# bminixhofer/zett

Measured on AMD Instinct MI355X. Metric: predicted token-embeddings/sec (full target vocab), higher is better.
Workload: dtype f16

## Files before the change

### zett_amd/csrc/gemm.hip.h

```cpp
#pragma once

#include <hip/hip_runtime.h>
#include <stdint.h>

#include <type_traits>

#ifndef ZETT_GROUP_M
#define ZETT_GROUP_M 4
#endif

namespace zett {

typedef __attribute__((ext_vector_type(16))) float f32x16;
typedef __attribute__((ext_vector_type(4))) float f32x4;
typedef __attribute__((ext_vector_type(8))) __bf16 bf16x8;
typedef __attribute__((ext_vector_type(4))) uint32_t u32x4;

typedef uint16_t bf16_t;
typedef _Float16 f16_t;
typedef __attribute__((ext_vector_type(8))) _Float16 f16x8;

__device__ __forceinline__ float bf16_to_f32(bf16_t v) { return __uint_as_float(((uint32_t)v) << 16); }
__device__ __forceinline__ bf16_t f32_to_bf16(float f) {
    return __builtin_bit_cast(bf16_t, (__bf16)f);
}

template <typename T> __device__ __forceinline__ T to_lo(float v);
template <> __device__ __forceinline__ float to_lo<float>(float v) { return v; }
template <> __device__ __forceinline__ bf16_t to_lo<bf16_t>(float v) { return f32_to_bf16(v); }
template <> __device__ __forceinline__ f16_t to_lo<f16_t>(float v) { return (f16_t)v; }
template <typename T> __device__ __forceinline__ float lo_to_f32(T v);
template <> __device__ __forceinline__ float lo_to_f32<float>(float v) { return v; }
template <> __device__ __forceinline__ float lo_to_f32<bf16_t>(bf16_t v) { return bf16_to_f32(v); }
template <> __device__ __forceinline__ float lo_to_f32<f16_t>(f16_t v) { return (float)v; }
template <typename T> __device__ __forceinline__ uint32_t pack2_lo(float a, float b);
template <> __device__ __forceinline__ uint32_t pack2_lo<bf16_t>(float a, float b) {
    typedef __attribute__((ext_vector_type(2))) float f32x2_t;
    typedef __attribute__((ext_vector_type(2))) __bf16 bf16x2_t;
    const f32x2_t v = {a, b};
    return __builtin_bit_cast(uint32_t, __builtin_convertvector(v, bf16x2_t));
}
template <> __device__ __forceinline__ uint32_t pack2_lo<f16_t>(float a, float b) {
    typedef __attribute__((ext_vector_type(2))) _Float16 h2;
    const h2 v = {(f16_t)a, (f16_t)b};
    return __builtin_bit_cast(uint32_t, v);
}
template <typename T> __device__ __forceinline__ void unpack2_lo(uint32_t u, float& a, float& b);
template <> __device__ __forceinline__ void unpack2_lo<bf16_t>(uint32_t u, float& a, float& b) { a = __uint_as_float(u << 16); b = __uint_as_float(u & 0xffff0000u); }
template <> __device__ __forceinline__ void unpack2_lo<f16_t>(uint32_t u, float& a, float& b) {
    typedef __attribute__((ext_vector_type(2))) _Float16 h2;
    const h2 v = __builtin_bit_cast(h2, u);
    a = (float)v[0]; b = (float)v[1];
}

enum { ACT_NONE = 0, ACT_GELU_TANH = 1, ACT_GELU_ERF = 2 };

__device__ __forceinline__ float gelu_tanh_f(float x) {
#pragma clang fp contract(off)
    const float x3 = (x * x) * x;
    const float u2 = 1.5957691216057308f * __builtin_fmaf(0.044715f, x3, x);
    const float t = 1.0f - 2.0f * __builtin_amdgcn_rcpf(1.0f + __builtin_amdgcn_exp2f(u2 * 1.4426950408889634f));
    return (0.5f * x) * (1.0f + t);
}
__device__ __forceinline__ float erf_as_f(float x) {
#pragma clang fp contract(off)
    const float ax = fabsf(x);
    const float t = __builtin_amdgcn_rcpf(__builtin_fmaf(0.3275911f, ax, 1.0f));
    float p = 1.061405429f;
    p = __builtin_fmaf(p, t, -1.453152027f);
    p = __builtin_fmaf(p, t, 1.421413741f);
    p = __builtin_fmaf(p, t, -0.284496736f);
    p = __builtin_fmaf(p, t, 0.254829592f);
    const float ex = __builtin_amdgcn_exp2f((ax * ax) * -1.4426950408889634f);
    const float y = __builtin_fmaf(-(p * t), ex, 1.0f);
    return copysignf(y, x);
}
__device__ __forceinline__ float gelu_erf_f(float x) {
#pragma clang fp contract(off)
    return (x * 0.5f) * (1.0f + erf_as_f(x * 0.70710678118654752440f));
}

__device__ __forceinline__ float ln_affine(float x, float mean, float rstd, float g, float b) {
#pragma clang fp contract(off)
    return __builtin_fmaf((x - mean) * rstd, g, b);
}

template <int ACT>
__device__ __forceinline__ float epi_value(float acc, float bias, bool has_res, float res, bool has_scale, float sc, float sh) {
#pragma clang fp contract(off)
    float v = acc + bias;
    if (ACT == 1) v = gelu_tanh_f(v);
    else if (ACT == 2) v = gelu_erf_f(v);
    if (has_res) v = v + res;
    if (has_scale) v = __builtin_fmaf(sc, v, sh);
    return v;
}
template <int ACT>
__device__ __forceinline__ float4 epi_value4(float4 a, float4 bias, bool has_res, float4 res, bool has_scale, float4 sc, float4 sh) {
    return make_float4(epi_value<ACT>(a.x, bias.x, has_res, res.x, has_scale, sc.x, sh.x), epi_value<ACT>(a.y, bias.y, has_res, res.y, has_scale, sc.y, sh.y),
                       epi_value<ACT>(a.z, bias.z, has_res, res.z, has_scale, sc.z, sh.z), epi_value<ACT>(a.w, bias.w, has_res, res.w, has_scale, sc.w, sh.w));
}

typedef __attribute__((ext_vector_type(2))) float f32x2;
#define ZETT_PIN_STAGE(arr, n) do { _Pragma("unroll") for (int e_ = 0; e_ < (n); ++e_) asm volatile("" : "+v"((arr)[e_])); } while (0)

template <int ACT, bool HAS_RES, bool HAS_SCALE, int NV>
__device__ __forceinline__ void epi_values(float (&vs)[NV], const float (&bias)[NV], const float (&res)[NV], const float (&sc)[NV], const float (&sh)[NV]) {
#pragma clang fp contract(off)
    static_assert(NV % 2 == 0, "pairs");
    constexpr int NP = NV / 2;
    f32x2 v[NP];
#pragma unroll
    for (int e = 0; e < NP; ++e) v[e] = f32x2{vs[2 * e], vs[2 * e + 1]} + f32x2{bias[2 * e], bias[2 * e + 1]};
    if (ACT == ACT_GELU_TANH) {
        f32x2 u2[NP], t[NP];
        ZETT_PIN_STAGE(v, NP);
#pragma unroll
        for (int e = 0; e < NP; ++e) u2[e] = (v[e] * v[e]) * v[e];
        ZETT_PIN_STAGE(u2, NP);
#pragma unroll
        for (int e = 0; e < NP; ++e) u2[e] = 1.5957691216057308f * __builtin_elementwise_fma(f32x2{0.044715f, 0.044715f}, u2[e], v[e]);
        ZETT_PIN_STAGE(u2, NP);
#pragma unroll
        for (int e = 0; e < NP; ++e) u2[e] = u2[e] * 1.4426950408889634f;
        ZETT_PIN_STAGE(u2, NP);
#pragma unroll
        for (int e = 0; e < NP; ++e) t[e] = f32x2{__builtin_amdgcn_exp2f(u2[e].x), __builtin_amdgcn_exp2f(u2[e].y)};
        ZETT_PIN_STAGE(t, NP);
#pragma unroll
        for (int e = 0; e < NP; ++e) t[e] = 1.0f + t[e];
        ZETT_PIN_STAGE(t, NP);
#pragma unroll
        for (int e = 0; e < NP; ++e) t[e] = f32x2{__builtin_amdgcn_rcpf(t[e].x), __builtin_amdgcn_rcpf(t[e].y)};
        ZETT_PIN_STAGE(t, NP);
#pragma unroll
        for (int e = 0; e < NP; ++e) t[e] = 1.0f - 2.0f * t[e];
        ZETT_PIN_STAGE(t, NP);
#pragma unroll
        for (int e = 0; e < NP; ++e) v[e] = (0.5f * v[e]) * (1.0f + t[e]);
        ZETT_PIN_STAGE(v, NP);
    } else if (ACT == ACT_GELU_ERF) {
        f32x2 z[NP], ax[NP], t[NP], p[NP], ex[NP];
        ZETT_PIN_STAGE(v, NP);
#pragma unroll
        for (int e = 0; e < NP; ++e) z[e] = v[e] * 0.70710678118654752440f;
        ZETT_PIN_STAGE(z, NP);
#pragma unroll
        for (int e = 0; e < NP; ++e) ax[e] = __builtin_elementwise_abs(z[e]);
#pragma unroll
        for (int e = 0; e < NP; ++e) t[e] = __builtin_elementwise_fma(f32x2{0.3275911f, 0.3275911f}, ax[e], f32x2{1.0f, 1.0f});
        ZETT_PIN_STAGE(t, NP);
#pragma unroll
        for (int e = 0; e < NP; ++e) t[e] = f32x2{__builtin_amdgcn_rcpf(t[e].x), __builtin_amdgcn_rcpf(t[e].y)};
        ZETT_PIN_STAGE(t, NP);
#pragma unroll
        for (int e = 0; e < NP; ++e) ex[e] = (ax[e] * ax[e]) * -1.4426950408889634f;
        ZETT_PIN_STAGE(ex, NP);
#pragma unroll
        for (int e = 0; e < NP; ++e) ex[e] = f32x2{__builtin_amdgcn_exp2f(ex[e].x), __builtin_amdgcn_exp2f(ex[e].y)};
        ZETT_PIN_STAGE(ex, NP);
#pragma unroll
        for (int e = 0; e < NP; ++e) p[e] = __builtin_elementwise_fma(f32x2{1.061405429f, 1.061405429f}, t[e], f32x2{-1.453152027f, -1.453152027f});
        ZETT_PIN_STAGE(p, NP);
#pragma unroll
        for (int e = 0; e < NP; ++e) p[e] = __builtin_elementwise_fma(p[e], t[e], f32x2{1.421413741f, 1.421413741f});
        ZETT_PIN_STAGE(p, NP);
#pragma unroll
        for (int e = 0; e < NP; ++e) p[e] = __builtin_elementwise_fma(p[e], t[e], f32x2{-0.284496736f, -0.284496736f});
        ZETT_PIN_STAGE(p, NP);
#pragma unroll
        for (int e = 0; e < NP; ++e) p[e] = __builtin_elementwise_fma(p[e], t[e], f32x2{0.254829592f, 0.254829592f});
        ZETT_PIN_STAGE(p, NP);
#pragma unroll
        for (int e = 0; e < NP; ++e) p[e] = -(p[e] * t[e]);
        ZETT_PIN_STAGE(p, NP);
#pragma unroll
        for (int e = 0; e < NP; ++e) p[e] = __builtin_elementwise_fma(p[e], ex[e], f32x2{1.0f, 1.0f});
        ZETT_PIN_STAGE(p, NP);
#pragma unroll
        for (int e = 0; e < NP; ++e) p[e] = 1.0f + __builtin_elementwise_copysign(p[e], z[e]);
        ZETT_PIN_STAGE(p, NP);
#pragma unroll
        for (int e = 0; e < NP; ++e) v[e] = (v[e] * 0.5f) * p[e];
        ZETT_PIN_STAGE(v, NP);
    }
    if (HAS_RES) {
#pragma unroll
        for (int e = 0; e < NP; ++e) v[e] = v[e] + f32x2{res[2 * e], res[2 * e + 1]};
    }
    if (HAS_SCALE) {
#pragma unroll
        for (int e = 0; e < NP; ++e) v[e] = __builtin_elementwise_fma(f32x2{sc[2 * e], sc[2 * e + 1]}, v[e], f32x2{sh[2 * e], sh[2 * e + 1]});
    }
#pragma unroll
    for (int e = 0; e < NP; ++e) { vs[2 * e] = v[e].x; vs[2 * e + 1] = v[e].y; }
}

template <typename T>
struct GemmEpilogue {
    const float* bias;
    int act;
    const float* residual;
    int ld_res;
    const float* res_stats;
    const float* res_gamma;
    const float* res_beta;
    const int32_t* res_index;
    float2* stats_part;
    int ld_part;
    const float* fold_stats;
    const float* fold_c;
    const float* scale;
    const float* shift;
    float* out_f32;
    int ld_f32;
    T* out_lo;
    int ld_lo;
    int split_col;
    float* out_f32_b;
    int32_t* range_flag;
    int range_final;
    const T* residual_lo;
    int ld_res_lo;
    void* dst;
    const int64_t* dst_rows;
    int64_t ld_dst;
    int dst_dtype;
};

template <typename T> struct LoRange { static constexpr bool checked = false; static constexpr float limit = 0.f; };
template <> struct LoRange<f16_t> { static constexpr bool checked = true; static constexpr float limit = 65504.0f; };
__device__ __forceinline__ bool out_of_range(float v, float limit) { return !(__builtin_fabsf(v) <= limit); }
constexpr float ZETT_F32_MAX = 3.402823466e38f;
constexpr int ZETT_RANGE_BIT_SOURCE = 1, ZETT_RANGE_BIT_ACTIVATION = 2, ZETT_RANGE_BIT_OUTPUT = 4, ZETT_RANGE_BIT_WEIGHT = 8, ZETT_RANGE_BIT_DEST = 16;
template <typename OT> __device__ __forceinline__ bool dest_overflow(float v) {
    if constexpr (std::is_same<OT, f16_t>::value) { const float a = __builtin_fabsf(v); return a >= 65520.0f && a <= 3.402823466e38f; }
    else return false;
// ... 201 lines not shown
```

### zett_amd/csrc/gemm4d.hip.h

```cpp
#pragma once

#include <hip/hip_runtime.h>
#include <stdint.h>

#include <algorithm>
#include <type_traits>

#include "gemm_tile.hip.h"

namespace zett {

#ifndef G4D_ABLATE
#define G4D_ABLATE 5
#endif
constexpr int G4D_ABL = G4D_ABLATE;
#ifdef G4D_MFMA32
constexpr bool G4D_M32 = true;
static_assert(G4D_ABLATE < 5, "the 32x32x16 K loop exists for the ablation levels without an epilogue");
#else
constexpr bool G4D_M32 = false;
#endif
typedef float f32x16 __attribute__((ext_vector_type(16)));

constexpr int g4d_wait_vm(int n) { return ((n >> 4) << 14) | 0x0F70 | (n & 15); }
// ... 14 lines not shown
    asm volatile("v_mfma_f32_32x32x16_f16 %0, %1, %2, %0" : "+a"(c) : "v"(a), "v"(b));
}

template <int K> __device__ __forceinline__ float g4d_xor_lane(float v) {
    return __builtin_bit_cast(float, __builtin_amdgcn_ds_swizzle(__builtin_bit_cast(int, v), (K << 10) | 0x1f));
}


enum { G4D_EPI_GENERIC = 0, G4D_EPI_LO = 1, G4D_EPI_F32 = 2, G4D_EPI_F32_SCALE = 3, G4D_EPI_BOTH = 4, G4D_EPI_F32_LN = 5, G4D_EPI_LO_FOLD = 6,
       G4D_EPI_LO_LN = 7, G4D_EPI_F32_SCALE_FOLD = 8, G4D_EPI_LN16 = 9 };
constexpr int G4D_EPI_STRIDE = 132;
constexpr int G4D_EPI_REGION = 64 * G4D_EPI_STRIDE * 4;
constexpr int G4D_LDS_BYTES = 4 * G4D_EPI_REGION;
static_assert(G4D_LDS_BYTES >= G256_LDS_BYTES && G4D_LDS_BYTES <= 160 * 1024, "LDS budget");

template <bool HALF> struct G4dGeom {
    static constexpr int BM = HALF ? 128 : G256_BM;
    static constexpr int WROWS = BM / 2;
    static constexpr int MI = WROWS / 16;
    static constexpr int AREQ = BM / 32;
    static constexpr int NREQ = AREQ + 8;
    static constexpr int NPASS = WROWS / 64;
    static constexpr int STAGES = HALF ? 3 : 2;
    static constexpr int A_BYTES = BM * GEMM_ROW_BYTES;
    static constexpr int STAGE_BYTES = A_BYTES + G256_OPERAND_BYTES;
    static constexpr int LDS_BYTES = STAGES * STAGE_BYTES;
};

template <typename T, int ACT = ACT_NONE, bool RES = false, int EPI = G4D_EPI_GENERIC, bool HALF = false, typename OT = void>
__global__ __launch_bounds__(256) __attribute__((amdgpu_waves_per_eu(1, 1))) void gemm4d_tn_kernel(GemmArgs<T> g) {
    extern __shared__ __attribute__((aligned(16))) unsigned char smem[];
    constexpr int BK = GEMM_ROW_BYTES / (int)sizeof(T);
    typedef G4dGeom<HALF> GEO;
    static_assert(!HALF || EPI != G4D_EPI_GENERIC, "the half tile carries the streamlined epilogues only");
    constexpr bool DST = !std::is_void<OT>::value;
    static_assert(!DST || EPI == G4D_EPI_F32_SCALE || EPI == G4D_EPI_F32_SCALE_FOLD, "destination stores: the output heads' epilogues only");

    const int tiles_m = (g.M - g.row0 + GEO::BM - 1) / GEO::BM;
    const int tiles_n = (g.N + G256_BN - 1) / G256_BN;
    const int nwg = tiles_m * tiles_n;
    int wg = blockIdx.x;
    {
        const int q = nwg >> 3, r = nwg & 7, xcd = wg & 7;
        wg = (xcd < r ? xcd * (q + 1) : r * (q + 1) + (xcd - r) * q) + (wg >> 3);
    }
    const int GROUP_N = g.group > 0 ? g.group : 4;
    int tm, tn;
    if (g.tile_order == 0) {
        const int group_size = GROUP_N * tiles_m;
        const int first_n = (wg / group_size) * GROUP_N;
        const int gn = (tiles_n - first_n) < GROUP_N ? (tiles_n - first_n) : GROUP_N;
        tn = first_n + (wg % group_size) % gn;
        tm = (wg % group_size) / gn;
    } else {
        const int GROUP_M = g.group > 0 ? g.group : ZETT_GROUP_M;
        const int group_size = GROUP_M * tiles_n;
        const int first_m = (wg / group_size) * GROUP_M;
        const int gm = (tiles_m - first_m) < GROUP_M ? (tiles_m - first_m) : GROUP_M;
        tm = first_m + (wg % group_size) % gm;
        tn = (wg % group_size) / gm;
    }
    const int m0 = g.row0 + tm * GEO::BM, n0 = tn * G256_BN;

    const int tid = threadIdx.x;
    const int lane = tid & 63;
    const int wave = __builtin_amdgcn_readfirstlane(tid >> 6);
    const int wm = wave >> 1, wn = wave & 1;

    const unsigned char* a_base = (const unsigned char*)(g.A + (size_t)m0 * g.lda);
    const unsigned char* w_base = (const unsigned char*)(g.W + (size_t)n0 * g.ldw);
    uint32_t a_voff[8], w_voff[8];
#pragma unroll
    for (int r = 0; r < 8; ++r) {
        const int row = wave * 64 + r * 8 + (lane >> 3);
        const int chunk = ((lane & 7) ^ ((row >> 1) & 7)) << 4;
        int wr = row; wr = n0 + wr < g.N ? wr : g.N - 1 - n0;
        w_voff[r] = (uint32_t)wr * (uint32_t)g.ldw * (uint32_t)sizeof(T) + chunk;
    }
#pragma unroll
    for (int r = 0; r < GEO::AREQ; ++r) {
        const int row = wave * (GEO::AREQ * 8) + r * 8 + (lane >> 3);
        const int chunk = ((lane & 7) ^ ((row >> 1) & 7)) << 4;
        int ar = row; ar = m0 + ar < g.M ? ar : g.M - 1 - m0;
        a_voff[r] = (uint32_t)ar * (uint32_t)g.lda * (uint32_t)sizeof(T) + chunk;
    }
    const __amdgpu_buffer_rsrc_t a_rsrc = __builtin_amdgcn_make_buffer_rsrc((void*)a_base, (short)0, 0x7fffffff, G4R_RSRC_WORD3);
    const __amdgpu_buffer_rsrc_t w_rsrc = __builtin_amdgcn_make_buffer_rsrc((void*)w_base, (short)0, 0x7fffffff, G4R_RSRC_WORD3);
    unsigned char* const my_rows = smem + wave * 64 * GEMM_ROW_BYTES;
    unsigned char* const my_a_rows = smem + wave * (GEO::AREQ * 8) * GEMM_ROW_BYTES;
    auto dma_a = [&](int stage, int kt, int r) {
        __builtin_amdgcn_raw_ptr_buffer_load_lds(a_rsrc, (lds_ptr_t)(my_a_rows + stage * GEO::STAGE_BYTES + r * 8 * GEMM_ROW_BYTES), 16,
                                                 a_voff[r], kt * GEMM_ROW_BYTES, 0, 0);
    };
    auto dma_w = [&](int stage, int kt, int r) {
        __builtin_amdgcn_raw_ptr_buffer_load_lds(w_rsrc, (lds_ptr_t)(my_rows + stage * GEO::STAGE_BYTES + GEO::A_BYTES + r * 8 * GEMM_ROW_BYTES), 16,
                                                 w_voff[r], kt * GEMM_ROW_BYTES, 0, 0);
    };

    constexpr bool M32 = G4D_M32 && !HALF;
    f32x4 acc[8][8];
    f32x16 acc32[4][4];
    if constexpr (M32) {
#pragma unroll
        for (int i = 0; i < 4; ++i)
#pragma unroll
            for (int j = 0; j < 4; ++j)
#pragma unroll
                for (int r = 0; r < 16; ++r) acc32[i][j][r] = 0.f;
    } else {
#pragma unroll
    for (int i = 0; i < GEO::MI; ++i)
#pragma unroll
        for (int j = 0; j < 8; ++j)
#pragma unroll
            for (int r = 0; r < 4; ++r) acc[i][j][r] = 0.f;
    }

    int a_off[2], w_off[2];
    {
        const int l15 = lane & 15, kq = lane >> 4;
        const int swz = (l15 >> 1) & 7;
#pragma unroll
        for (int kb = 0; kb < 2; ++kb) {
            const int c = ((kb * 4 + kq) ^ swz) << 4;
            a_off[kb] = (wm * GEO::WROWS + l15) * GEMM_ROW_BYTES + c;
            w_off[kb] = GEO::A_BYTES + (wn * 128 + l15) * GEMM_ROW_BYTES + c;
        }
    }
    int a_off32[4], w_off32[4];
    if constexpr (M32) {
        const int l31 = lane & 31, kh = lane >> 5;
        const int swz = (l31 >> 1) & 7;
#pragma unroll
        for (int k16 = 0; k16 < 4; ++k16) {
            const int c = ((k16 * 2 + kh) ^ swz) << 4;
            a_off32[k16] = (wm * GEO::WROWS + l31) * GEMM_ROW_BYTES + c;
            w_off32[k16] = GEO::A_BYTES + (wn * 128 + l31) * GEMM_ROW_BYTES + c;
        }
    }
    u32x4 fa[2][8], fw[2][8];
    auto read_a = [&](int stage, int kb, int i) {
        if constexpr (M32) fa[kb][i] = *(const u32x4*)(smem + stage * GEO::STAGE_BYTES + a_off32[kb * 2 + (i >> 2)] + (i & 3) * 32 * GEMM_ROW_BYTES);
        else fa[kb][i] = *(const u32x4*)(smem + stage * GEO::STAGE_BYTES + a_off[kb] + i * 16 * GEMM_ROW_BYTES);
    };
    auto read_w = [&](int stage, int kb, int j) {
        if constexpr (M32) fw[kb][j] = *(const u32x4*)(smem + stage * GEO::STAGE_BYTES + w_off32[kb * 2 + (j >> 2)] + (j & 3) * 32 * GEMM_ROW_BYTES);
        else fw[kb][j] = *(const u32x4*)(smem + stage * GEO::STAGE_BYTES + w_off[kb] + j * 16 * GEMM_ROW_BYTES);
    };

    const int nk = g.K / BK;
    constexpr bool LN16K = EPI == G4D_EPI_LN16;
    uint4 res16[LN16K ? 16 : 1];
    const bool res16_early = LN16K && g.epi.res_index == nullptr;
    auto res16_request = [&](int p, int t) __attribute__((always_inline)) {
        if constexpr (LN16K) {
            int grow = m0 + wm * GEO::WROWS + p * 64 + t * 4 + (lane >> 4);
            grow = grow < g.M ? grow : g.M - 1;
            int gc = n0 + wn * 128 + (lane & 15) * 8;
            gc = gc < g.N ? gc : 0;
            res16[t] = *(const uint4*)(g.epi.residual_lo + (size_t)grow * g.epi.ld_res_lo + gc);
        }
    };
#pragma unroll
    for (int st = 0; st < GEO::STAGES; ++st) {
        if (st < nk) {
#pragma unroll
            for (int r = 0; r < 8; ++r) dma_w(st, st, r);
#pragma unroll
            for (int r = 0; r < GEO::AREQ; ++r) dma_a(st, st, r);
        }
    }
    {
        const int ahead = (nk < GEO::STAGES ? nk : GEO::STAGES) - 1;
        if (ahead >= 2) __builtin_amdgcn_s_waitcnt(g4d_wait_vm(2 * GEO::NREQ));
        else if (ahead == 1) __builtin_amdgcn_s_waitcnt(g4d_wait_vm(GEO::NREQ));
        else __builtin_amdgcn_s_waitcnt(g4d_wait_vm(0));
    }
    __builtin_amdgcn_s_barrier();
    __builtin_amdgcn_sched_barrier(0);
#pragma unroll
    for (int j = 0; j < 8; ++j) read_w(0, 0, j);
#pragma unroll
    for (int i = 0; i < GEO::MI; ++i) read_a(0, 0, i);
    if constexpr (G4D_ABL < 2) {
#pragma unroll
        for (int j = 0; j < 8; ++j) read_w(0, 1, j);
#pragma unroll
        for (int i = 0; i < GEO::MI; ++i) read_a(0, 1, i);
        __builtin_amdgcn_s_waitcnt(G4R_WAIT_LGKM0);
    }

    auto step = [&](int kt, int cur, auto more_c, auto more2_c, auto moreA_c, auto wave_c) {
        constexpr bool more = decltype(more_c)::value, more2 = decltype(more2_c)::value, moreA = decltype(moreA_c)::value;
        constexpr int WV = decltype(wave_c)::value;
        const int nxt = cur + 1 == GEO::STAGES ? 0 : cur + 1;
        constexpr int P_BAR1 = HALF ? 26 : 36, P_BAR2 = HALF ? 52 : 102;
        constexpr int INFLIGHT = HALF ? ((more2 ? 1 : 0) + (moreA ? 1 : 0)) * GEO::NREQ : (moreA ? GEO::NREQ : 0);
#pragma unroll
        for (int kb = 0; kb < 2; ++kb)
#pragma unroll
        for (int i = 0; i < GEO::MI; ++i)
#pragma unroll
        for (int j = 0; j < 8; ++j) {
            const int p = kb * (GEO::MI * 8) + i * 8 + j;
            if (G4D_ABL >= 4 && p == P_BAR1 && (moreA || (!more && EPI != G4D_EPI_GENERIC))) {
                __builtin_amdgcn_s_waitcnt(G4R_WAIT_LGKM0);
                __builtin_amdgcn_s_barrier();
                __builtin_amdgcn_sched_barrier(0);
            }
            if (G4D_ABL >= 4 && p == P_BAR2 && more) {
                __builtin_amdgcn_s_waitcnt(g4d_wait_vm(INFLIGHT));
                __builtin_amdgcn_s_barrier();
                __builtin_amdgcn_sched_barrier(0);
            }
            if constexpr (M32) {
                if ((p & 1) == 0) {
                    const int q = (p >> 1) & 31, h = q >> 4, i32 = (q >> 2) & 3, j32 = q & 3;
                    mfma32_agpr<T>(acc32[i32][j32], fa[kb][h * 4 + i32], fw[kb][h * 4 + j32]);
                }
            } else
            mfma16_agpr<T>(acc[i][j], fa[kb][i], fw[kb][j]);
            constexpr bool RD = G4D_ABL >= 2, DMA = G4D_ABL >= 3;
            if (RD && p < 16 && (p & 1) == 0) read_w(cur, 1, p >> 1);
            if constexpr (!HALF) {
                if (RD && p >= 16 && p <= 30 && (p & 1) == 0) read_a(cur, 1, (p - 16) >> 1);
                if (DMA && moreA && p >= 38 && p < 70 && WV == ((p - 38) & 3)) dma_w(cur, kt + 2, (p - 38) >> 2);
                if (DMA && moreA && p >= 70 && p < 102 && WV == ((p - 70) & 3)) dma_a(cur, kt + 2, (p - 70) >> 2);
                if (RD && more && p >= 103 && p <= 110) read_w(nxt, 0, p - 103);
                if (RD && more && p >= 111 && p <= 125 && (p & 1) == 1) read_a(nxt, 0, (p - 111) >> 1);
                if constexpr (LN16K) { if (!more && p >= 40 && p < 104 && (p & 3) == 0 && res16_early) res16_request(0, (p - 40) >> 2); }
            } else {
                if (p >= 16 && p <= 22 && (p & 1) == 0) read_a(cur, 1, (p - 16) >> 1);
                if (moreA && p >= 27 && p < 43 && (WV & 1) == ((p - 27) & 1)) dma_w(cur, kt + 3, (p - 27) >> 1);
                if (moreA && p >= 43 && p < 51 && (WV & 1) == ((p - 43) & 1)) dma_a(cur, kt + 3, (p - 43) >> 1);
                if (more && p >= 53 && p <= 60) read_w(nxt, 0, p - 53);
                if (more && p >= 60 && p <= 63) read_a(nxt, 0, p - 60);
                if constexpr (LN16K) { if (!more && p >= 24 && p < 56 && (p & 1) == 0 && res16_early) res16_request(0, (p - 24) >> 1); }
            }
            if (!M32 || (p & 1)) __builtin_amdgcn_sched_barrier(0);
        }
    };
    typedef std::integral_constant<bool, true> yes_t;
    typedef std::integral_constant<bool, false> no_t;
    auto k_loop = [&](auto wave_c) {
        int kt = 0, cur = 0;
        auto next = [&]() { ++kt; cur = cur + 1 == GEO::STAGES ? 0 : cur + 1; };
        for (; kt + GEO::STAGES < nk; next()) step(kt, cur, yes_t{}, yes_t{}, yes_t{}, wave_c);
        if constexpr (HALF) {
            if (kt + 2 < nk) { step(kt, cur, yes_t{}, yes_t{}, no_t{}, wave_c); next(); }
        }
        if (kt + 1 < nk) { step(kt, cur, yes_t{}, no_t{}, no_t{}, wave_c); next(); }
        step(kt, cur, no_t{}, no_t{}, no_t{}, wave_c);
    };
    if (wave == 0) k_loop(std::integral_constant<int, 0>{});
    else if (wave == 1) k_loop(std::integral_constant<int, 1>{});
    else if (wave == 2) k_loop(std::integral_constant<int, 2>{});
    else k_loop(std::integral_constant<int, 3>{});

    asm volatile("s_nop 15\n\ts_nop 15");
    if constexpr (G4D_ABL < 5) {
        float keep = 0.f;
        if constexpr (M32) {
#pragma unroll
            for (int i = 0; i < 4; ++i)
#pragma unroll
                for (int j = 0; j < 4; ++j)
#pragma unroll
                    for (int r = 0; r < 16; ++r) keep += acc32[i][j][r];
        } else {
#pragma unroll
        for (int i = 0; i < GEO::MI; ++i)
#pragma unroll
            for (int j = 0; j < 8; ++j) keep += acc[i][j][0] + acc[i][j][1] + acc[i][j][2] + acc[i][j][3];
        }
        if (keep == 123.456f) g.epi.out_lo[threadIdx.x] = (T)0;
        return;
    }
    int tid_e = tid;
    asm volatile("" : "+v"(tid_e));
    const int lane_e = tid_e & 63;
    const int l15 = lane_e & 15, kq = lane_e >> 4;
    if constexpr (EPI == G4D_EPI_GENERIC) {
        __syncthreads();
        float* region = (float*)(smem + wave * 32768);
        typedef EpiDrain<T, ACT, RES, 64, 128, !RES, false> Drain;
        const int gcol = n0 + wn * 128 + (lane_e % Drain::LPR) * 8;
        const bool col_ok = gcol < g.N;
        float4 bias8[2], sc8[2], sh8[2];
        Drain::load_cols(g.epi, gcol, col_ok, bias8, sc8, sh8);
        float4 lng[2], lnb[2];
        Drain::load_ln_cols(g.epi, gcol, col_ok, lng, lnb);
#pragma unroll
        for (int p = 0; p < 2; ++p) {
            float4 oa[Drain::NIT], ob[Drain::NIT];
            const int row0 = m0 + wm * 128 + p * 64;
            Drain::load_res(g, row0, gcol, col_ok, lane_e, oa, ob);
            float2 lnst;
            Drain::load_res_stats(g, row0, lane_e, lnst);
#pragma unroll
            for (int i4 = 0; i4 < 4; ++i4)
#pragma unroll
                for (int j = 0; j < 8; ++j)
#pragma unroll
                    for (int r = 0; r < 4; ++r)
                        region[(i4 * 16 + kq * 4 + r) * 128 + j * 16 + l15] = acc[4 * p + i4][j][r];
            if (RES || p == 0) __builtin_amdgcn_s_waitcnt(GEMM_WAIT_VMCNT0);
            Drain::ln_res(g, lane_e, lng, lnb, lnst, oa, ob);
            Drain::drain(g, region, row0, gcol, col_ok, lane_e, bias8, sc8, sh8, oa, ob);
        }
    } else {
        constexpr bool LO = EPI == G4D_EPI_LO || EPI == G4D_EPI_LO_FOLD, SCALE = EPI == G4D_EPI_F32_SCALE || EPI == G4D_EPI_F32_SCALE_FOLD;
        constexpr bool LN16 = EPI == G4D_EPI_LN16;
        constexpr bool LNP = EPI == G4D_EPI_F32_LN || EPI == G4D_EPI_LO_LN || LN16, FOLD = EPI == G4D_EPI_LO_FOLD || EPI == G4D_EPI_F32_SCALE_FOLD;
        constexpr bool WF32 = EPI != G4D_EPI_LO_LN && !LN16;
        static_assert(!LNP || RES, "a LayerNorm producer is a residual epilogue");
        static_assert((EPI != G4D_EPI_F32_LN && !LN16) || ACT == ACT_NONE, "the encoder's producer has no activation");
        static_assert(!LN16 || sizeof(T) == 2, "16-bit residual stream");
        constexpr int CPL = (LO || LN16) ? 8 : 4;
        constexpr int LPR = 128 / CPL;
        constexpr int RPI = 64 / LPR;
        constexpr int NIT = 64 / RPI;
        static_assert(!(LO && RES), "the 16-bit-only epilogue has no residual");
        float* region = (float*)(smem + wave * G4D_EPI_REGION);
        const GemmEpilogue<T>& e = g.epi;
        constexpr bool W16 = LO || EPI == G4D_EPI_BOTH || LNP;
        constexpr bool CHK16 = W16 && LoRange<T>::checked;
        const bool chk_final = !W16 && e.range_final != 0;
        bool bad = false;
        const int idx = lane_e % LPR, rsub = lane_e / LPR;
        const int gcol = n0 + wn * 128 + idx * CPL;
        const bool col_ok = gcol < g.N;
        const int grow0 = m0 + wm * GEO::WROWS + rsub;
        float bias[CPL], sc[CPL], sh[CPL];
#pragma unroll
        for (int c = 0; c < CPL; ++c) { bias[c] = 0.f; sc[c] = 1.f; sh[c] = 0.f; }
        if (col_ok) {
#pragma unroll
            for (int c4 = 0; c4 < CPL; c4 += 4) {
                if (e.bias) { const float4 b = *(const float4*)(e.bias + gcol + c4); bias[c4] = b.x; bias[c4 + 1] = b.y; bias[c4 + 2] = b.z; bias[c4 + 3] = b.w; }
                if (SCALE) {
                    const float4 a = *(const float4*)(e.scale + gcol + c4), b = *(const float4*)(e.shift + gcol + c4);
                    sc[c4] = a.x; sc[c4 + 1] = a.y; sc[c4 + 2] = a.z; sc[c4 + 3] = a.w;
                    sh[c4] = b.x; sh[c4 + 1] = b.y; sh[c4 + 2] = b.z; sh[c4 + 3] = b.w;
                }
            }
        }
        const bool res_ln = RES && ACT == ACT_NONE && e.res_stats != nullptr;
        float lg[CPL], lb[CPL];
#pragma unroll
        for (int c = 0; c < CPL; ++c) { lg[c] = 1.f; lb[c] = 0.f; }
        float2 pst[2] = {make_float2(0.f, 1.f), make_float2(0.f, 1.f)};
        if constexpr (RES && ACT == ACT_NONE) {
            if (res_ln) {
                if (col_ok) {
#pragma unroll
                    for (int c4 = 0; c4 < CPL; c4 += 4) {
                        const float4 a = *(const float4*)(e.res_gamma + gcol + c4), b = *(const float4*)(e.res_beta + gcol + c4);
                        lg[c4] = a.x; lg[c4 + 1] = a.y; lg[c4 + 2] = a.z; lg[c4 + 3] = a.w; lb[c4] = b.x; lb[c4 + 1] = b.y; lb[c4 + 2] = b.z; lb[c4 + 3] = b.w;
                    }
                }
#pragma unroll
                for (int p = 0; p < GEO::NPASS; ++p) {
                    int srow = m0 + wm * GEO::WROWS + p * 64 + lane_e; srow = srow < g.M ? srow : g.M - 1;
                    if (e.res_index) srow = e.res_index[srow];
                    pst[p] = *(const float2*)(e.res_stats + 2 * (size_t)srow);
                }
            }
        }
        int rix[2] = {0, 0};
        const bool res_ix = RES && e.res_index != nullptr;
        if constexpr (RES) {
            if (res_ix) {
#pragma unroll
                for (int p = 0; p < GEO::NPASS; ++p) {
                    int srow = m0 + wm * GEO::WROWS + p * 64 + lane_e; srow = srow < g.M ? srow : g.M - 1;
                    rix[p] = e.res_index[srow];
                }
            }
        }
        float fc[FOLD ? CPL : 1];
        float2 fst[2] = {make_float2(0.f, 1.f), make_float2(0.f, 1.f)};
        if constexpr (FOLD) {
#pragma unroll
            for (int c = 0; c < CPL; ++c) fc[c] = 0.f;
            if (col_ok) {
#pragma unroll
                for (int c4 = 0; c4 < CPL; c4 += 4) {
                    const float4 a = *(const float4*)(e.fold_c + gcol + c4);
                    fc[c4] = a.x; fc[c4 + 1] = a.y; fc[c4 + 2] = a.z; fc[c4 + 3] = a.w;
                }
            }
#pragma unroll
            for (int p = 0; p < GEO::NPASS; ++p) {
                int srow = m0 + wm * GEO::WROWS + p * 64 + lane_e; srow = srow < g.M ? srow : g.M - 1;
                fst[p] = *(const float2*)(e.fold_stats + 2 * (size_t)srow);
            }
        }
        int64_t drow[2] = {0, 0};
        if constexpr (DST) {
#pragma unroll
            for (int p = 0; p < GEO::NPASS; ++p) {
                int srow = m0 + wm * GEO::WROWS + p * 64 + lane_e; srow = srow < g.M ? srow : g.M - 1;
                drow[p] = e.dst_rows ? e.dst_rows[srow] : (int64_t)srow;
            }
        }
        bool bad_dst = false;
        constexpr int RB = LNP ? 1 : 2;
        float4 res[LN16 ? 1 : RB][(RES && !LN16) ? NIT : 1];
        auto load_res16 = [&](int p, int ta, int tb) {
            if constexpr (LN16) {
#pragma unroll
                for (int t = ta; t < tb; ++t) {
                    if (res_ix) {
                        const int grow = grow0 + p * 64 + t * RPI;
                        const size_t rrow = (size_t)__shfl(rix[p], t * RPI + rsub, 64);
                        res16[t] = (grow < g.M && col_ok) ? *(const uint4*)(e.residual_lo + rrow * e.ld_res_lo + gcol) : make_uint4(0u, 0u, 0u, 0u);
                    } else {
                        res16_request(p, t);
                    }
                }
            }
        };
        auto load_res = [&](int p) {
            if constexpr (LN16) {
                load_res16(p, 0, NIT);
            } else if constexpr (RES) {
#pragma unroll
                for (int t = 0; t < NIT; ++t) {
                    const int grow = grow0 + p * 64 + t * RPI;
                    size_t rrow = (size_t)grow;
                    if (res_ix) {
                        const int i0 = __builtin_amdgcn_readlane(rix[p], t * RPI), i1 = __builtin_amdgcn_readlane(rix[p], t * RPI + 1);
                        rrow = (size_t)(rsub ? i1 : i0);
                    }
                    res[p % RB][t] = (grow < g.M && col_ok) ? *(const float4*)(e.residual + rrow * e.ld_res + gcol) : make_float4(0.f, 0.f, 0.f, 0.f);
                }
            }
        };
        auto stage = [&](int p) {
#pragma unroll
            for (int i4 = 0; i4 < 4; ++i4)
#pragma unroll
                for (int j = 0; j < 8; ++j)
#pragma unroll
                    for (int r = 0; r < 4; ++r)
                        region[(i4 * 16 + kq * 4 + r) * G4D_EPI_STRIDE + j * 16 + l15] = acc[4 * p + i4][j][r];
            if constexpr (FOLD)
                *(float2*)(region + lane_e * G4D_EPI_STRIDE + 128) = fst[p];
            if constexpr (LN16)
                *(float2*)(region + lane_e * G4D_EPI_STRIDE + 128) = pst[p];
        };
        auto drain = [&](int p, auto full_c) {
            constexpr bool FULL = decltype(full_c)::value;
            constexpr int GROUP = (LO || RES) ? 4 : 8;
            constexpr int NV = GROUP * CPL;
            float acc_s = 0.f, acc_q = 0.f;
#pragma unroll
            for (int t0 = 0; t0 < NIT; t0 += GROUP) {
                float v[NV], bb[NV], rr[NV], ss[NV], hh[NV];
#pragma unroll
                for (int u = 0; u < GROUP; ++u) {
                    const float* src = region + ((t0 + u) * RPI + rsub) * G4D_EPI_STRIDE + idx * CPL;
#pragma unroll
                    for (int c4 = 0; c4 < CPL; c4 += 4) {
                        const float4 x = *(const float4*)(src + c4);
                        v[u * CPL + c4] = x.x; v[u * CPL + c4 + 1] = x.y; v[u * CPL + c4 + 2] = x.z; v[u * CPL + c4 + 3] = x.w;
                    }
#pragma unroll
                    for (int c = 0; c < CPL; ++c) { bb[u * CPL + c] = bias[c]; ss[u * CPL + c] = sc[c]; hh[u * CPL + c] = sh[c]; rr[u * CPL + c] = 0.f; }
                    if constexpr (LN16) {
                        const uint4 x = res16[t0 + u];
                        unpack2_lo<T>(x.x, rr[u * 8], rr[u * 8 + 1]); unpack2_lo<T>(x.y, rr[u * 8 + 2], rr[u * 8 + 3]);
                        unpack2_lo<T>(x.z, rr[u * 8 + 4], rr[u * 8 + 5]); unpack2_lo<T>(x.w, rr[u * 8 + 6], rr[u * 8 + 7]);
                        if (res_ln) {
                            const float2 st = *(const float2*)(region + ((t0 + u) * RPI + rsub) * G4D_EPI_STRIDE + 128);
#pragma unroll
                            for (int c = 0; c < 8; ++c) rr[u * 8 + c] = ln_affine(rr[u * 8 + c], st.x, st.y, lg[c], lb[c]);
                        }
                    } else if constexpr (RES) {
                        const float4 x = res[p % RB][t0 + u];
                        rr[u * CPL] = x.x; rr[u * CPL + 1] = x.y; rr[u * CPL + 2] = x.z; rr[u * CPL + 3] = x.w;
                        if (ACT == ACT_NONE && res_ln) {
                            const int r0 = (t0 + u) * RPI;
                            const float mean0 = __builtin_bit_cast(float, __builtin_amdgcn_readlane(__builtin_bit_cast(int, pst[p].x), r0));
                            const float mean1 = __builtin_bit_cast(float, __builtin_amdgcn_readlane(__builtin_bit_cast(int, pst[p].x), r0 + 1));
                            const float rstd0 = __builtin_bit_cast(float, __builtin_amdgcn_readlane(__builtin_bit_cast(int, pst[p].y), r0));
                            const float rstd1 = __builtin_bit_cast(float, __builtin_amdgcn_readlane(__builtin_bit_cast(int, pst[p].y), r0 + 1));
                            const float mean = rsub ? mean1 : mean0, rstd = rsub ? rstd1 : rstd0;
#pragma unroll
                            for (int c = 0; c < 4; ++c) rr[u * CPL + c] = ln_affine(rr[u * CPL + c], mean, rstd, lg[c], lb[c]);
                        }
                    }
                }
                if constexpr (FOLD) {
#pragma unroll
                    for (int u = 0; u < GROUP; ++u) {
                        const float2 st = *(const float2*)(region + ((t0 + u) * RPI + rsub) * G4D_EPI_STRIDE + 128);
                        const float t = -st.x * st.y;
                        const f32x2 t2 = {t, t}, r2 = {st.y, st.y};
#pragma unroll
                        for (int c = 0; c < CPL; c += 2) {
                            const f32x2 x = __builtin_elementwise_fma(t2, f32x2{fc[c], fc[c + 1]}, f32x2{bias[c], bias[c + 1]});
                            const f32x2 y = __builtin_elementwise_fma(f32x2{v[u * CPL + c], v[u * CPL + c + 1]}, r2, x);
                            v[u * CPL + c] = y.x; v[u * CPL + c + 1] = y.y;
                            bb[u * CPL + c] = 0.f; bb[u * CPL + c + 1] = 0.f;
                        }
                    }
                }
                epi_values<ACT, RES, SCALE, NV>(v, bb, rr, ss, hh);
                if constexpr (CHK16) {
#pragma unroll
                    for (int x = 0; x < NV; ++x) bad |= out_of_range(v[x], LoRange<T>::limit);
                } else if (chk_final) {
#pragma unroll
                    for (int x = 0; x < NV; ++x) bad |= out_of_range(v[x], ZETT_F32_MAX);
                }
                if constexpr (LN16) {
                    static_assert(!LN16 || (GROUP == 4 && CPL == 8 && RPI == 4), "reduce-scatter layout");
                    float S[4], Q[4];
#pragma unroll
                    for (int u = 0; u < 4; ++u) {
                        const float* x = v + 8 * u;
                        S[u] = ((x[0] + x[1]) + (x[2] + x[3])) + ((x[4] + x[5]) + (x[6] + x[7]));
                        Q[u] = __builtin_fmaf(x[0], x[0], __builtin_fmaf(x[1], x[1], __builtin_fmaf(x[2], x[2], __builtin_fmaf(x[3], x[3],
                               __builtin_fmaf(x[4], x[4], __builtin_fmaf(x[5], x[5], __builtin_fmaf(x[6], x[6], x[7] * x[7])))))));
                    }
                    const bool b3 = (idx & 8) != 0, b2 = (idx & 4) != 0;
                    float ks0 = b3 ? S[2] : S[0], ks1 = b3 ? S[3] : S[1], kq0 = b3 ? Q[2] : Q[0], kq1 = b3 ? Q[3] : Q[1];
                    ks0 += g4d_xor_lane<8>(b3 ? S[0] : S[2]); ks1 += g4d_xor_lane<8>(b3 ? S[1] : S[3]);
                    kq0 += g4d_xor_lane<8>(b3 ? Q[0] : Q[2]); kq1 += g4d_xor_lane<8>(b3 ? Q[1] : Q[3]);
                    float ks = b2 ? ks1 : ks0, kq = b2 ? kq1 : kq0;
                    ks += g4d_xor_lane<4>(b2 ? ks0 : ks1); kq += g4d_xor_lane<4>(b2 ? kq0 : kq1);
                    ks += g4d_xor_lane<2>(ks); kq += g4d_xor_lane<2>(kq);
                    ks += g4d_xor_lane<1>(ks); kq += g4d_xor_lane<1>(kq);
                    const bool mine = (idx & 3) == (t0 >> 2);
                    acc_s = mine ? ks : acc_s; acc_q = mine ? kq : acc_q;
                } else if constexpr (LNP) {
                    static_assert(GROUP == 4 && CPL == 4 && RPI == 2, "reduce-scatter layout");
                    float S[4], Q[4];
#pragma unroll
                    for (int u = 0; u < 4; ++u) {
                        const float a = v[4 * u], b = v[4 * u + 1], c = v[4 * u + 2], d = v[4 * u + 3];
                        S[u] = (a + b) + (c + d);
                        Q[u] = __builtin_fmaf(a, a, __builtin_fmaf(b, b, __builtin_fmaf(c, c, d * d)));
                    }
                    const bool b4 = (idx & 16) != 0, b3 = (idx & 8) != 0;
                    float ks0 = b4 ? S[2] : S[0], ks1 = b4 ? S[3] : S[1], kq0 = b4 ? Q[2] : Q[0], kq1 = b4 ? Q[3] : Q[1];
                    ks0 += g4d_xor_lane<16>(b4 ? S[0] : S[2]); ks1 += g4d_xor_lane<16>(b4 ? S[1] : S[3]);
                    kq0 += g4d_xor_lane<16>(b4 ? Q[0] : Q[2]); kq1 += g4d_xor_lane<16>(b4 ? Q[1] : Q[3]);
                    float ks = b3 ? ks1 : ks0, kq = b3 ? kq1 : kq0;
                    ks += g4d_xor_lane<8>(b3 ? ks0 : ks1); kq += g4d_xor_lane<8>(b3 ? kq0 : kq1);
                    ks += g4d_xor_lane<4>(ks); kq += g4d_xor_lane<4>(kq);
                    ks += g4d_xor_lane<2>(ks); kq += g4d_xor_lane<2>(kq);
                    ks += g4d_xor_lane<1>(ks); kq += g4d_xor_lane<1>(kq);
                    const bool mine = (idx & 7) == (t0 >> 2);
                    acc_s = mine ? ks : acc_s; acc_q = mine ? kq : acc_q;
                }
#pragma unroll
                for (int u = 0; u < GROUP; ++u) {
                    const int grow = grow0 + p * 64 + (t0 + u) * RPI;
                    if (!FULL && (grow >= g.M || !col_ok)) continue;
                    if constexpr (LO || LN16) {
                        const float4 a = make_float4(v[u * 8], v[u * 8 + 1], v[u * 8 + 2], v[u * 8 + 3]);
                        const float4 b = make_float4(v[u * 8 + 4], v[u * 8 + 5], v[u * 8 + 6], v[u * 8 + 7]);
                        store_out8<T>(e.out_lo + (size_t)grow * e.ld_lo + gcol, a, b);
                    } else {
                        const f32x4 x = {v[u * 4], v[u * 4 + 1], v[u * 4 + 2], v[u * 4 + 3]};
                        if constexpr (DST) {
                            const int r0 = (t0 + u) * RPI;
                            static_assert(!DST || RPI == 2, "two rows per instruction");
                            const uint64_t d64 = (uint64_t)drow[p];
                            const uint32_t lo0 = __builtin_amdgcn_readlane((uint32_t)d64, r0), hi0 = __builtin_amdgcn_readlane((uint32_t)(d64 >> 32), r0);
                            const uint32_t lo1 = __builtin_amdgcn_readlane((uint32_t)d64, r0 + 1), hi1 = __builtin_amdgcn_readlane((uint32_t)(d64 >> 32), r0 + 1);
                            const int64_t d = (int64_t)(((uint64_t)(rsub ? hi1 : hi0) << 32) | (rsub ? lo1 : lo0));
                            if (d >= 0) {
                                store_out4<OT>((OT*)e.dst + d * e.ld_dst + gcol, make_float4(x[0], x[1], x[2], x[3]));
#pragma unroll
                                for (int c = 0; c < 4; ++c) bad_dst |= dest_overflow<OT>(x[c]);
                            }
                        } else if constexpr (WF32) {
                            float* d = e.out_f32 + (size_t)grow * e.ld_f32 + gcol;
                            if (RES) asm volatile("global_store_dwordx4 %0, %1, off nt\n\ts_nop 1" :: "v"(d), "v"(x) : "memory");
                            else *(f32x4*)d = x;
                        }
                        if constexpr (EPI == G4D_EPI_BOTH || LNP)
                            store_out4<T>(e.out_lo + (size_t)grow * e.ld_lo + gcol, make_float4(x[0], x[1], x[2], x[3]));
                    }
                }
                if constexpr (LN16 && GEO::NPASS == 2) { if (p == 0 && t0 == GROUP) load_res16(1, 0, NIT / 2); }
            }
            if constexpr (LN16 && GEO::NPASS == 2) { if (p == 0) load_res16(1, NIT / 2, NIT); }
            if constexpr (LNP) {
                const int rp = LN16 ? (((4 * (idx & 3) + 2 * ((idx >> 3) & 1) + ((idx >> 2) & 1)) << 2) + rsub)
                                    : (((4 * (idx & 7) + 2 * ((idx >> 4) & 1) + ((idx >> 3) & 1)) << 1) + rsub);
                const int grow = m0 + wm * GEO::WROWS + p * 64 + rp;
                if (grow < g.M && n0 + wn * 128 < g.N)
                    e.stats_part[(size_t)((n0 + wn * 128) >> 7) * e.ld_part + grow] = make_float2(acc_s, acc_q);
            }
        };
        auto drain_pass = [&](int p) {
            const bool full = m0 + wm * GEO::WROWS + p * 64 + 64 <= g.M && n0 + wn * 128 + 128 <= g.N;
            if (full) drain(p, std::integral_constant<bool, true>{});
            else drain(p, std::integral_constant<bool, false>{});
        };
        if constexpr (LN16) { if (!res16_early) load_res(0); }
        else load_res(0);
        stage(0);
        __builtin_amdgcn_sched_barrier(0);
        if constexpr (!LNP && GEO::NPASS == 2) load_res(1);
        __builtin_amdgcn_sched_barrier(0);
        drain_pass(0);
        if constexpr (GEO::NPASS == 2) {
            if constexpr (LNP && !LN16) { __builtin_amdgcn_sched_barrier(0); load_res(1); __builtin_amdgcn_sched_barrier(0); }
            stage(1);
            drain_pass(1);
        }
        range_report(e.range_flag, bad, W16 ? ZETT_RANGE_BIT_ACTIVATION : ZETT_RANGE_BIT_OUTPUT);
        if constexpr (DST) range_report(e.range_flag, bad_dst, ZETT_RANGE_BIT_DEST);
    }
}

template <typename T>
inline int gemm4d_epi_mode(const GemmArgs<T>& g) {
    const GemmEpilogue<T>& e = g.epi;
    if (e.stats_part && e.residual_lo) {
        if (sizeof(T) == 2 && e.out_lo && !e.out_f32 && !e.residual && e.act == ACT_NONE && !e.scale && !e.shift && !e.out_f32_b && e.split_col >= g.N &&
            g.N % 128 == 0 && e.ld_lo % 8 == 0 && e.ld_res_lo % 8 == 0) return G4D_EPI_LN16;
        return -1;
    }
    if (e.stats_part) {
        const bool common = e.out_lo && e.residual && !e.scale && !e.shift && !e.out_f32_b && e.split_col >= g.N && g.N % 128 == 0 &&
                            e.ld_lo % 4 == 0 && e.ld_res % 4 == 0;
        if (common && e.out_f32 && e.act == ACT_NONE && e.ld_f32 % 4 == 0) return G4D_EPI_F32_LN;
        if (common && !e.out_f32 && e.act == ACT_GELU_TANH && !e.res_stats && !e.res_index) return G4D_EPI_LO_LN;
        return -1;
    }
    if (e.fold_stats) {
        if (e.fold_c && e.out_lo && !e.out_f32 && !e.residual && !e.scale && !e.shift && !e.out_f32_b && e.split_col >= g.N &&
            g.N % 8 == 0 && e.ld_lo % 8 == 0) return G4D_EPI_LO_FOLD;
        if (e.fold_c && e.out_f32 && !e.out_lo && !e.residual && e.scale && e.shift && e.act == ACT_NONE && !e.out_f32_b && e.split_col >= g.N &&
            g.N % 4 == 0 && e.ld_f32 % 4 == 0) return G4D_EPI_F32_SCALE_FOLD;
        return -1;
    }
    if (e.out_f32_b || e.split_col < g.N) return G4D_EPI_GENERIC;
    if (e.res_stats && (e.act != ACT_NONE || !e.residual)) return G4D_EPI_GENERIC;
    if (e.out_lo && !e.out_f32 && !e.residual && !e.scale && !e.shift && g.N % 8 == 0 && e.ld_lo % 8 == 0) return G4D_EPI_LO;
    if (e.out_f32 && e.out_lo && !e.residual && !e.scale && !e.shift && e.act == ACT_NONE && g.N % 4 == 0 && e.ld_f32 % 4 == 0 && e.ld_lo % 4 == 0)
        return G4D_EPI_BOTH;
    if (e.out_f32 && !e.out_lo && g.N % 4 == 0 && e.ld_f32 % 4 == 0 && (!e.residual || e.ld_res % 4 == 0)) {
        if (e.scale && e.shift && !e.residual && e.act == ACT_NONE) return G4D_EPI_F32_SCALE;
        if (!e.scale && !e.shift && (e.act == ACT_NONE || (e.act == ACT_GELU_TANH && e.residual))) return G4D_EPI_F32;
    }
    return G4D_EPI_GENERIC;
}

template <typename T, int ACT, bool RES, int EPI, bool HALF = false>
inline hipError_t launch_gemm4d_inst(const GemmArgs<T>& g, hipStream_t stream) {
    constexpr int lds = EPI == G4D_EPI_GENERIC ? G256_LDS_BYTES : (G4dGeom<HALF>::LDS_BYTES > G4D_LDS_BYTES ? G4dGeom<HALF>::LDS_BYTES : G4D_LDS_BYTES);
    static_assert(lds <= 160 * 1024, "LDS budget");
    static DeviceFlags attr;
    bool* done = attr.current();
    if (!done || !*done) {
        hipError_t e = hipFuncSetAttribute((const void*)gemm4d_tn_kernel<T, ACT, RES, EPI, HALF>, hipFuncAttributeMaxDynamicSharedMemorySize, lds);
        if (e != hipSuccess) return e;
        if (done) *done = true;
    }
    constexpr int BM = HALF ? 128 : G256_BM;
    const int tiles_m = (g.M - g.row0 + BM - 1) / BM;
    const int tiles_n = (g.N + G256_BN - 1) / G256_BN;
    if (tiles_m <= 0 || tiles_n <= 0) return hipSuccess;
    hipLaunchKernelGGL((gemm4d_tn_kernel<T, ACT, RES, EPI, HALF>), dim3(tiles_m * tiles_n), dim3(256), lds, stream, g);
    return hipGetLastError();
}

template <typename T, int ACT, bool HALF>
inline hipError_t launch_gemm4d_act(const GemmArgs<T>& g, hipStream_t stream, int mode) {
    const bool res = g.epi.residual != nullptr;
    switch (mode) {
        case G4D_EPI_LO: return launch_gemm4d_inst<T, ACT, false, G4D_EPI_LO, HALF>(g, stream);
        case G4D_EPI_LO_FOLD: return launch_gemm4d_inst<T, ACT, false, G4D_EPI_LO_FOLD, HALF>(g, stream);
        case G4D_EPI_F32:
            if constexpr (ACT == ACT_NONE) return res ? launch_gemm4d_inst<T, ACT, true, G4D_EPI_F32, HALF>(g, stream) : launch_gemm4d_inst<T, ACT, false, G4D_EPI_F32, HALF>(g, stream);
            else if constexpr (ACT == ACT_GELU_TANH) { if (res) return launch_gemm4d_inst<T, ACT, true, G4D_EPI_F32, HALF>(g, stream); }
            [[fallthrough]];
        default:
            if constexpr (HALF) return hipErrorInvalidValue;
            else return res ? launch_gemm4d_inst<T, ACT, true, G4D_EPI_GENERIC>(g, stream) : launch_gemm4d_inst<T, ACT, false, G4D_EPI_GENERIC>(g, stream);
    }
}

template <typename T, bool HALF>
inline hipError_t launch_gemm4d_mode(const GemmArgs<T>& g, hipStream_t stream, int mode) {
    if (mode == G4D_EPI_F32_LN) return launch_gemm4d_inst<T, ACT_NONE, true, G4D_EPI_F32_LN, HALF>(g, stream);
    if (mode == G4D_EPI_LN16) return launch_gemm4d_inst<T, ACT_NONE, true, G4D_EPI_LN16, HALF>(g, stream);
    if (mode == G4D_EPI_LO_LN) return launch_gemm4d_inst<T, ACT_GELU_TANH, true, G4D_EPI_LO_LN, HALF>(g, stream);
    if (mode == G4D_EPI_F32_SCALE_FOLD) return launch_gemm4d_inst<T, ACT_NONE, false, G4D_EPI_F32_SCALE_FOLD, HALF>(g, stream);
    if (mode == G4D_EPI_F32_SCALE) return launch_gemm4d_inst<T, ACT_NONE, false, G4D_EPI_F32_SCALE, HALF>(g, stream);
    if (mode == G4D_EPI_BOTH) return launch_gemm4d_inst<T, ACT_NONE, false, G4D_EPI_BOTH, HALF>(g, stream);
    switch (g.epi.act) {
        case ACT_GELU_TANH: return launch_gemm4d_act<T, ACT_GELU_TANH, HALF>(g, stream, mode);
        case ACT_GELU_ERF: return launch_gemm4d_act<T, ACT_GELU_ERF, HALF>(g, stream, mode);
        default: return launch_gemm4d_act<T, ACT_NONE, HALF>(g, stream, mode);
    }
}

template <typename T>
inline bool gemm4d_half_ok(const GemmArgs<T>& g, int mode) {
    if (mode <= G4D_EPI_GENERIC) return false;
    if (mode == G4D_EPI_F32) return g.epi.act == ACT_NONE || (g.epi.act == ACT_GELU_TANH && g.epi.residual);
    return true;
}

inline int gemm4d_row_split(int M, int N, int cus = 256, double half_cost = 0.62) {
    const long tn = (N + G256_BN - 1) / G256_BN, tm = (M + G256_BM - 1) / G256_BM;
    const long T = tm * tn;
    if (T % cus == 0) return M;
    const long rounds = (T + cus - 1) / cus;
    const long tm_full = std::min<long>(tm, ((rounds - 1) * cus) / tn);
    const long row0 = tm_full * G256_BM;
    if (row0 >= M) return M;
    const long th = ((M - row0 + 127) / 128) * tn;
    const double cost = (double)((tm_full * tn + cus - 1) / cus) + half_cost * (double)((th + cus - 1) / cus);
    return cost < (double)rounds - 0.05 ? (int)row0 : M;
}

template <typename T, int EPI, typename OT, bool HALF>
inline hipError_t launch_gemm4d_dst_inst(const GemmArgs<T>& g, hipStream_t stream) {
    constexpr int lds = G4dGeom<HALF>::LDS_BYTES > G4D_LDS_BYTES ? G4dGeom<HALF>::LDS_BYTES : G4D_LDS_BYTES;
    static DeviceFlags attr;
    bool* done = attr.current();
    if (!done || !*done) {
        hipError_t e = hipFuncSetAttribute((const void*)gemm4d_tn_kernel<T, ACT_NONE, false, EPI, HALF, OT>, hipFuncAttributeMaxDynamicSharedMemorySize, lds);
        if (e != hipSuccess) return e;
        if (done) *done = true;
    }
    constexpr int BM = HALF ? 128 : G256_BM;
    const int tiles_m = (g.M - g.row0 + BM - 1) / BM;
    const int tiles_n = (g.N + G256_BN - 1) / G256_BN;
    if (tiles_m <= 0 || tiles_n <= 0) return hipSuccess;
    hipLaunchKernelGGL((gemm4d_tn_kernel<T, ACT_NONE, false, EPI, HALF, OT>), dim3(tiles_m * tiles_n), dim3(256), lds, stream, g);
    return hipGetLastError();
}

template <typename T, bool HALF>
inline hipError_t launch_gemm4d_dst_mode(const GemmArgs<T>& g, hipStream_t stream, int mode) {
    const int dt = g.epi.dst_dtype;
    if (mode == G4D_EPI_F32_SCALE_FOLD) {
        if (dt == 1) return launch_gemm4d_dst_inst<T, G4D_EPI_F32_SCALE_FOLD, f16_t, HALF>(g, stream);
        if (dt == 2) return launch_gemm4d_dst_inst<T, G4D_EPI_F32_SCALE_FOLD, bf16_t, HALF>(g, stream);
        return launch_gemm4d_dst_inst<T, G4D_EPI_F32_SCALE_FOLD, float, HALF>(g, stream);
    }
    if (dt == 1) return launch_gemm4d_dst_inst<T, G4D_EPI_F32_SCALE, f16_t, HALF>(g, stream);
    if (dt == 2) return launch_gemm4d_dst_inst<T, G4D_EPI_F32_SCALE, bf16_t, HALF>(g, stream);
    return launch_gemm4d_dst_inst<T, G4D_EPI_F32_SCALE, float, HALF>(g, stream);
}

template <typename T>
inline int gemm4d_dst_mode(const GemmArgs<T>& g) {
    const GemmEpilogue<T>& e = g.epi;
    if (!e.dst || e.dst_dtype < 0 || e.dst_dtype > 2 || e.ld_dst % 4 != 0) return -1;
    const size_t align = e.dst_dtype == 0 ? 16 : 8;
    if ((uintptr_t)e.dst % align) return -1;
    GemmArgs<T> f = g;
    f.epi.out_f32 = (float*)e.dst;
    f.epi.ld_f32 = 4;
    const int mode = gemm4d_epi_mode(f);
    return (mode == G4D_EPI_F32_SCALE || mode == G4D_EPI_F32_SCALE_FOLD) ? mode : -1;
}

hipError_t launch_gemm_4d_half(const GemmArgs<f16_t>& g, hipStream_t stream, int mode);
hipError_t launch_gemm_4d_half(const GemmArgs<bf16_t>& g, hipStream_t stream, int mode);

hipError_t launch_gemm_4d_half_dst(const GemmArgs<f16_t>& g, hipStream_t stream, int mode);
hipError_t launch_gemm_4d_half_dst(const GemmArgs<bf16_t>& g, hipStream_t stream, int mode);

template <typename T>
inline hipError_t launch_gemm4d(const GemmArgs<T>& g, hipStream_t stream, bool force_generic = false) {
    const bool dst = g.epi.dst != nullptr;
    const int mode = dst ? gemm4d_dst_mode(g) : (force_generic && !g.epi.stats_part && !g.epi.fold_stats) ? G4D_EPI_GENERIC : gemm4d_epi_mode(g);
    if (mode < 0) return hipErrorInvalidValue;
    int split = g.row0 == -1 ? gemm4d_row_split(g.M, g.N) : (g.row0 == -2 ? 0 : (g.row0 > 0 ? std::min(g.row0, g.M) : g.M));
    if (split < g.M && (!gemm4d_half_ok(g, mode) || split % G256_BM != 0)) split = g.M;
    GemmArgs<T> full = g;
    full.row0 = 0;
    if (split < g.M) {
        full.M = split;
        if (split > 0)
            if (hipError_t e = dst ? launch_gemm4d_dst_mode<T, false>(full, stream, mode) : launch_gemm4d_mode<T, false>(full, stream, mode); e != hipSuccess) return e;
        GemmArgs<T> rest = g;
        rest.row0 = split;
        return dst ? launch_gemm_4d_half_dst(rest, stream, mode) : launch_gemm_4d_half(rest, stream, mode);
    }
    return dst ? launch_gemm4d_dst_mode<T, false>(full, stream, mode) : launch_gemm4d_mode<T, false>(full, stream, mode);
}

}
```

### zett_amd/csrc/rowops.hip.h

```cpp
#pragma once

#include <hip/hip_runtime.h>
#include <stdint.h>

#include <type_traits>

#include "gemm.hip.h"

namespace zett {


struct PlanArrays {
    int32_t* row_count;
    int32_t* row_offset;
    uint8_t* row_uniform;
    int32_t* id_flag;
    int32_t* id_slot;
    int32_t* id_list;
    int32_t* tok_slot;
    int32_t* tok_pos;
    int32_t* tok_row;
    int32_t* tok_pkey;
    int32_t* pair_flag;
    int32_t* pair_slot;
// ... 600 lines not shown

struct AttentionWaves { int64_t total, full; int full_groups, lanes_per_row; };
__host__ __device__ inline AttentionWaves attention_waves(int rows, int H, bool pack) {
    const int rem = H & 511, gfull = H >> 9;
    AttentionWaves a;
    if (pack && (rem == 256 || rem == 128 || rem == 64)) {
        a.full_groups = gfull; a.lanes_per_row = rem >> 3;
        a.full = (int64_t)rows * gfull;
        const int per = 64 / a.lanes_per_row;
        a.total = a.full + (rows + per - 1) / per;
    } else {
        a.full_groups = (H + 511) >> 9; a.lanes_per_row = 64;
        a.full = (int64_t)rows * a.full_groups;
        a.total = a.full;
    }
    return a;
}

template <typename T>
__global__ __launch_bounds__(256) void attention_rows_kernel(const T* __restrict__ qbase, size_t ldq,
                                                             const T* __restrict__ kbase, const T* __restrict__ vbase,
                                                             size_t ldkv, int H, int head_dim,
                                                             const int32_t* __restrict__ row_offset,
                                                             const uint8_t* __restrict__ row_uniform,
                                                             const uint8_t* __restrict__ tok_key, int64_t row0,
                                                             int rows, int tok0, float scaling, int flags ,
                                                             const int32_t* __restrict__ tok_pair, T* __restrict__ ctx) {
    const int cls_only = flags & 1;
    const int lane = threadIdx.x & 63;
    const int64_t w = (int64_t)blockIdx.x * 4 + (threadIdx.x >> 6);
    const AttentionWaves aw = attention_waves(rows, H, (flags & 4) != 0);
    if (w >= aw.total) return;
    int rl, grp, li = lane, base = 0, lpr = 64;
    bool valid = true;
    if (w < aw.full) { rl = (int)(w / aw.full_groups); grp = (int)(w % aw.full_groups); }
    else {
        lpr = aw.lanes_per_row;
        const int sub = lane / lpr;
        li = lane - sub * lpr;
        base = sub * lpr;
        rl = (int)(w - aw.full) * (64 / lpr) + sub;
        grp = aw.full_groups;
        valid = rl < rows;
        if (!valid) rl = rows - 1;
    }
    const int col = grp * 512 + li * 8;
    const bool active = valid && col < H;
    const int lph = head_dim >> 3;
    const int64_t n = row0 + rl;
    const int t0 = row_offset[n] - tok0, t1 = row_offset[n + 1] - tok0;
    const bool uniform = row_uniform[n];
    const int nq = cls_only ? 1 : (t1 - t0);
    const int ccol = active ? col : 0;
    auto brow = [&](int t) -> size_t { return (size_t)chunk_row(t, rl, t == t0, rows); };
    int pslot = 0;
    if (tok_pair) { const int t = t0 + li; pslot = t < t1 ? tok_pair[tok0 + t] : 0; }
    auto qrow = [&](int t) -> size_t {
        if (!tok_pair) return brow(t);
        return t - t0 < lpr ? (size_t)__shfl(pslot, base + (t - t0), 64) : (size_t)tok_pair[tok0 + t];
    };
    const int nk = t1 - t0;
    if constexpr (sizeof(T) == 2) {
        if (nk <= ATT_FAST_KEYS && (flags & 2)) {
            const bool mine = li < nk && (uniform || tok_key[tok0 + t0 + li] != 0);
            const unsigned on = (unsigned)(__ballot(mine) >> base) & (lpr >= 32 ? 0xffffffffu : ((1u << lpr) - 1u));
            uint4 kk[ATT_FAST_KEYS], vv[ATT_FAST_KEYS], qq[ATT_FAST_KEYS];
#pragma unroll
            for (int j = 0; j < ATT_FAST_KEYS; ++j) {
                if (j < nk) {
                    const size_t kr = qrow(t0 + j);
                    kk[j] = *(const uint4*)(kbase + kr * ldkv + ccol);
                    vv[j] = *(const uint4*)(vbase + kr * ldkv + ccol);
                    if (!cls_only) qq[j] = *(const uint4*)(qbase + kr * ldq + ccol);
                }
            }
            if (cls_only) qq[0] = *(const uint4*)(qbase + (size_t)rl * ldq + ccol);
            const float sc2 = scaling * 1.4426950408889634f;
#pragma unroll
            for (int qi = 0; qi < ATT_FAST_KEYS; ++qi) {
                if (qi < nq) {
                    float sj[ATT_FAST_KEYS];
                    float mx = -INFINITY;
#pragma unroll
                    for (int j = 0; j < ATT_FAST_KEYS; ++j) {
                        sj[j] = -INFINITY;
                        if (j < nk && ((on >> j) & 1u)) {
                            const float d = head_sum(dot8_lo<T>(qq[qi], kk[j]), lph);
                            sj[j] = uniform ? 0.f : d * sc2;
                            mx = fmaxf(mx, sj[j]);
                        }
                    }
                    float l = 0.f, acc[8];
#pragma unroll
                    for (int c = 0; c < 8; ++c) acc[c] = 0.f;
#pragma unroll
                    for (int j = 0; j < ATT_FAST_KEYS; ++j) {
                        if (j < nk && ((on >> j) & 1u)) {
                            const float pj = __builtin_amdgcn_exp2f(sj[j] - mx);
                            l += pj;
                            float v[8];
                            unpack2_lo<T>(vv[j].x, v[0], v[1]); unpack2_lo<T>(vv[j].y, v[2], v[3]);
                            unpack2_lo<T>(vv[j].z, v[4], v[5]); unpack2_lo<T>(vv[j].w, v[6], v[7]);
#pragma unroll
                            for (int c = 0; c < 8; ++c) acc[c] = fmaf(pj, v[c], acc[c]);
                        }
                    }
                    const float inv = 1.0f / l;
#pragma unroll
                    for (int c = 0; c < 8; ++c) acc[c] *= inv;
                    if (active) {
                        const size_t orow = cls_only ? (size_t)rl : brow(t0 + qi);
                        store8<T>(ctx + orow * H + col, acc);
                    }
                }
            }
            return;
        }
    }
    for (int qi = 0; qi < nq; ++qi) {
        float q[8];
        load8<T>(qbase + (cls_only ? (size_t)rl : qrow(t0 + qi)) * ldq + ccol, q);
        float mx = -INFINITY, l = 0.f, acc[8];
#pragma unroll
        for (int c = 0; c < 8; ++c) acc[c] = 0.f;
        for (int kj = t0; kj < t1; ++kj) {
            if (!uniform && !tok_key[tok0 + kj]) continue;
            float k[8], v[8];
            const size_t kr = qrow(kj);
            load8<T>(kbase + kr * ldkv + ccol, k);
            load8<T>(vbase + kr * ldkv + ccol, v);
            float s = 0.f;
#pragma unroll
            for (int c = 0; c < 8; ++c) s = fmaf(q[c], k[c], s);
            for (int off = 1; off < lph; off <<= 1) s += __shfl_xor(s, off, 64);
            s = uniform ? 0.f : s * scaling;
            const float nm = fmaxf(mx, s);
            const float corr = expf(mx - nm);
            const float p = expf(s - nm);
            l = fmaf(l, corr, p);
#pragma unroll
            for (int c = 0; c < 8; ++c) acc[c] = fmaf(acc[c], corr, p * v[c]);
            mx = nm;
        }
        const float inv = 1.0f / l;
#pragma unroll
        for (int c = 0; c < 8; ++c) acc[c] *= inv;
        if (active) {
            const size_t orow = cls_only ? (size_t)rl : brow(t0 + qi);
            store8<T>(ctx + orow * H + col, acc);
        }
    }
}

__global__ __launch_bounds__(64) void ln_stats_kernel(const float2* __restrict__ part, int parts, int ld_part, int rows, int H, float eps,
                                                      float* __restrict__ stats) {
    const int r = blockIdx.x * blockDim.x + threadIdx.x;
    if (r >= rows) return;
    float s = 0.f, q = 0.f;
    const float2* col = part + r;
    int p = 0;
    for (; p + 8 <= parts; p += 8) {
        float2 v[8];
#pragma unroll
        for (int j = 0; j < 8; ++j) v[j] = col[(size_t)(p + j) * ld_part];
#pragma unroll
        for (int j = 0; j < 8; ++j) { s += v[j].x; q += v[j].y; }
    }
    {
        float2 v[8];
#pragma unroll
        for (int j = 0; j < 8; ++j) v[j] = p + j < parts ? col[(size_t)(p + j) * ld_part] : make_float2(0.f, 0.f);
#pragma unroll
        for (int j = 0; j < 8; ++j)
            if (p + j < parts) { s += v[j].x; q += v[j].y; }
    }
    const float mean = s / (float)H;
    const float var = fmaxf(q / (float)H - mean * mean, 0.f);
    *(float2*)(stats + 2 * (size_t)r) = make_float2(mean, 1.0f / sqrtf(var + eps));
}

template <typename T>
__global__ __launch_bounds__(256) void fold_weight_kernel(const float* __restrict__ w, int K, const float* __restrict__ gamma,
                                                          const float* __restrict__ beta, const float* __restrict__ bias,
                                                          T* __restrict__ w_fold, float* __restrict__ c_out, float* __restrict__ b_out,
                                                          int32_t* __restrict__ range_flag) {
    __shared__ float red[4];
    const int n = blockIdx.x;
    const float* row = w + (size_t)n * K;
    float cs = 0.f, bs = 0.f;
    for (int k = threadIdx.x; k < K; k += 256) {
        const float x = row[k];
        if (LoRange<T>::checked) range_report(range_flag, out_of_range(x * gamma[k], LoRange<T>::limit), ZETT_RANGE_BIT_WEIGHT);
        const T lo = to_lo<T>(x * gamma[k]);
        w_fold[(size_t)n * K + k] = lo;
        cs += lo_to_f32<T>(lo);
        bs = fmaf(x, beta[k], bs);
    }
    const float ct = block_sum_256(cs, red);
    const float bt = block_sum_256(bs, red);
    if (threadIdx.x == 0) { c_out[n] = ct; b_out[n] = bias[n] + bt; }
}

template <typename T>
__global__ void convert_f32_to_lo_kernel(const float* __restrict__ in, T* __restrict__ out, size_t n, int32_t* __restrict__ range_flag) {
    size_t i = ((size_t)blockIdx.x * blockDim.x + threadIdx.x) * 4;
    const size_t stride = (size_t)gridDim.x * blockDim.x * 4;
    bool bad = false;
    for (; i + 3 < n; i += stride) {
        const float4 v = *(const float4*)(in + i);
        if (LoRange<T>::checked)
            bad |= out_of_range(v.x, LoRange<T>::limit) | out_of_range(v.y, LoRange<T>::limit) | out_of_range(v.z, LoRange<T>::limit) |
                   out_of_range(v.w, LoRange<T>::limit);
        store_lo4<T>(out + i, v);
    }
    if (blockIdx.x == 0 && threadIdx.x == 0) {
        for (size_t j = n & ~(size_t)3; j < n; ++j) { out[j] = to_lo<T>(in[j]); if (LoRange<T>::checked) bad |= out_of_range(in[j], LoRange<T>::limit); }
    }
    range_report(range_flag, bad, ZETT_RANGE_BIT_WEIGHT);
}
template <int SRC_DTYPE>
__global__ void convert_to_f32_kernel(const void* __restrict__ in, float* __restrict__ out, size_t n) {
    size_t i = (size_t)blockIdx.x * blockDim.x + threadIdx.x;
    const size_t stride = (size_t)gridDim.x * blockDim.x;
    for (; i < n; i += stride) {
        if constexpr (SRC_DTYPE == 1) out[i] = (float)((const _Float16*)in)[i];
        else out[i] = __uint_as_float(((uint32_t)((const uint16_t*)in)[i]) << 16);
    }
}

template <typename OT> __device__ __forceinline__ void store4_dst(OT* d, float4 v) {
    if constexpr (std::is_same<OT, float>::value) *(float4*)d = v;
    else *(uint2*)d = make_uint2(pack2_lo<OT>(v.x, v.y), pack2_lo<OT>(v.z, v.w));
}

template <typename OT, bool VEC>
__global__ __launch_bounds__(256) void dest_store_rows_kernel(const float* __restrict__ src, int64_t ld_src, OT* __restrict__ dst, int64_t ld_dst,
                                                              const int64_t* __restrict__ rows, int64_t n_rows, int cols, int32_t* range_flag) {
    bool bad = false;
    for (int64_t i = blockIdx.x; i < n_rows; i += gridDim.x) {
        const int64_t d = rows ? rows[i] : i;
        if (d < 0) continue;
        const float* s = src + i * ld_src;
        OT* o = dst + d * ld_dst;
        if constexpr (VEC) {
            for (int c = (int)threadIdx.x * 4; c < cols; c += 256 * 4) {
                const float4 v = *(const float4*)(s + c);
                store4_dst<OT>(o + c, v);
                bad |= dest_overflow<OT>(v.x) | dest_overflow<OT>(v.y) | dest_overflow<OT>(v.z) | dest_overflow<OT>(v.w);
            }
        } else {
            for (int c = (int)threadIdx.x; c < cols; c += 256) {
                const float v = s[c];
                o[c] = to_lo<OT>(v);
                bad |= dest_overflow<OT>(v);
            }
        }
    }
    range_report(range_flag, bad, ZETT_RANGE_BIT_DEST);
}

__global__ void dest_rows_check_kernel(const int64_t* __restrict__ rows, int64_t n, int64_t n_dest, int32_t* err) {
    const int64_t i = (int64_t)blockIdx.x * blockDim.x + threadIdx.x;
    if (i < n && rows[i] >= n_dest) atomicMax(err, (int)(i < 0x7ffffffe ? i + 1 : 0x7fffffff));
}

}
```

### zett_amd/csrc/zett_hip.hip

```cpp
#include <hip/hip_runtime.h>

#include <algorithm>
#include <array>
#include <cstdlib>
#include <cmath>
#include <cstdarg>
#include <cstdio>
#include <cstring>
#include <map>
#include <string>
#include <type_traits>
#include <vector>

#include "../../include/zett_hip.h"
#include "common.hip.h"
#include "gemm.hip.h"
#include "gemm_launch.hip.h"
#include "rowops.hip.h"
#include "retok.hip.h"
#include "lexical.hip.h"
#include "partition.hip.h"

using namespace zett;

namespace {

struct Tensor {
    float* f32 = nullptr;
    void* lo = nullptr;
    std::vector<int64_t> shape;
    size_t numel = 0;
};

inline size_t round_up(size_t v, size_t m) { return (v + m - 1) / m * m; }

}

struct zett_hypernet {
    zett_config cfg{};
    int device = 0;
    int precision = ZETT_PREC_BF16;
    bool finalized = false;
    std::map<std::string, Tensor> w;
    std::vector<void*> qkv_w;
    std::vector<float*> qkv_b;
    struct Folded { void* w = nullptr; float* c = nullptr; float* b = nullptr; };
    std::vector<Folded> fold_qkv, fold_up;
    Folded fold_head_in, fold_head_out;
    float* head_one = nullptr;
    float* head_zero = nullptr;
    int ln_fold = 1;
    float* head_scale = nullptr;
    float* head_shift = nullptr;
    std::vector<void*> owned;
    int64_t max_chunk_tokens = 0;
    int time_gemm = 0;
    int cls_only_last = 1;
    int pair_dedupe = 1;
    int residual_lo = 1;
    int concurrent_lanes = 0;
    hipStream_t lane_stream = nullptr;
    hipEvent_t lane_ev[4] = {nullptr, nullptr, nullptr, nullptr};
    int attention_fast = 1;
    int attention_pack = 1;
    int gemm_tail_split = 1;
    int gemm_tile_order = 0;
    int ln_rows8 = 1;
    int table_lo = 1;
    int gemm_group = 0;
    int gemm4d_min_k = 512;
    int gemm_variant = 0;
    struct PlanSlot {
        DevBuf i32, u8;
        int32_t* host = nullptr;
        size_t host_ints = 0;
        hipEvent_t done = nullptr;
        hipEvent_t released = nullptr;
        const int32_t* sfm = nullptr;
        int64_t n_rows = 0;
        int seq = 0;
        bool pair_plan = false;
        const int32_t* ext_id_slot = nullptr;
        bool pending = false;
    } plan[2];
    PlanSlot table_plan;
    struct ExtTable { const void* table = nullptr; const float* stats = nullptr; const int32_t* id_slot = nullptr; } ext;
    int plan_cur = 0;
    hipStream_t plan_stream = nullptr;
    hipEvent_t plan_fork = nullptr;
    DevBuf table, x0, yf, yt, big, pre, ctx, cf, ct, lnstats, lnparts;
    hipEvent_t out_ready[2] = {nullptr, nullptr};
    bool out_recorded = false;
    int range_accumulate = 0;
    int32_t* range_word = nullptr;
    int32_t* range_host = nullptr;
    DevBuf dest_word, dest_stage[2], dest_sink;
    int32_t* dest_host = nullptr;
    hipEvent_t dest_checked = nullptr;
    std::vector<hipEvent_t> ev;
    size_t ev_used = 0;
    std::vector<double> ev_flops;
    std::vector<std::array<int, 4>> ev_shape;
    std::vector<zett_gemm_record> gemm_log;
    zett_stats stats{};
};

namespace {

size_t elt_size(int precision) { return precision == ZETT_PREC_F32 ? 4 : 2; }

bool is_gemm_weight(const std::string& n) {
    static const char* suffixes[] = {"input_projection.0.weight", "dense1.weight", "dense2.weight",
                                     "query.weight", "key.weight", "value.weight", "dense.weight",
                                     "output_projection.1.weight", "output_projection_out.1.weight"};
    for (const char* s : suffixes) {
        const size_t ls = strlen(s);
        if (n.size() >= ls && n.compare(n.size() - ls, ls, s) == 0) return true;
    }
    return false;
}

void expected_shapes(const zett_config& c, std::map<std::string, std::vector<int64_t>>& s) {
    const int64_t H = c.hidden, I = c.intermediate;
    auto proj = [&](const std::string& p) {
        s[p + "dense1.weight"] = {I, H}; s[p + "dense1.bias"] = {I};
        s[p + "dense2.weight"] = {H, I}; s[p + "dense2.bias"] = {H};
        s[p + "ln.weight"] = {H}; s[p + "ln.bias"] = {H};
    };
    if (c.embed_lang) s["lang_embeddings.weight"] = {c.n_langs, H};
    s["model.embeddings.token_type_embeddings.weight"] = {1, H};
    s["model.embeddings.LayerNorm.weight"] = {H};
    s["model.embeddings.LayerNorm.bias"] = {H};
    s["model.embeddings.position_embeddings.weight"] = {c.max_positions, H};
    for (int l = 0; l < c.layers; ++l) {
        const std::string p = "model.encoder.layer." + std::to_string(l) + ".";
        for (const char* q : {"query", "key", "value"}) {
            s[p + "attention.self." + q + ".weight"] = {H, H};
            s[p + "attention.self." + q + ".bias"] = {H};
        }
        s[p + "attention.output.dense.weight"] = {H, H}; s[p + "attention.output.dense.bias"] = {H};
        s[p + "attention.output.LayerNorm.weight"] = {H}; s[p + "attention.output.LayerNorm.bias"] = {H};
        s[p + "intermediate.dense.weight"] = {I, H}; s[p + "intermediate.dense.bias"] = {I};
        s[p + "output.dense.weight"] = {H, I}; s[p + "output.dense.bias"] = {H};
        s[p + "output.LayerNorm.weight"] = {H}; s[p + "output.LayerNorm.bias"] = {H};
    }
    s["fallback_embeddings.weight"] = {c.n_extra, c.n_in_embd};
    s["input_projection.0.weight"] = {H, c.n_in_embd}; s["input_projection.0.bias"] = {H};
    proj("input_projection.1.");
    proj("output_projection.0.");
    const int64_t w0 = c.single_head ? c.n_in_embd : c.n_embd;
    s["output_projection.1.weight"] = {w0, H}; s["output_projection.1.bias"] = {w0};
    if (c.separate_out && !c.single_head) {
        proj("output_projection_out.0.");
        s["output_projection_out.1.weight"] = {c.n_embd, H}; s["output_projection_out.1.bias"] = {c.n_embd};
    }
    if (c.rescale) {
        s["in_scaler.w"] = {1, c.n_in_embd}; s["in_scaler.b"] = {1, c.n_in_embd};
        s["scaler.w"] = {1, c.n_embd}; s["scaler.b"] = {1, c.n_embd};
        if (c.separate_out) { s["out_scaler.w"] = {1, c.n_embd}; s["out_scaler.b"] = {1, c.n_embd}; }
    }
    if (c.predict_bias) { s["bias_projection.weight"] = {1, H}; s["bias_projection.bias"] = {1}; }
}

int validate_config(const zett_config& c, int precision) {
    if (c.n_embd <= 0 || c.hidden <= 0 || c.intermediate <= 0 || c.heads <= 0 || c.layers <= 0)
        return fail(ZETT_E_INVALID, "non-positive dimension in zett_config");
    if (c.n_in_embd != (c.separate_out ? 2 * c.n_embd : c.n_embd))
        return fail(ZETT_E_INVALID, "n_in_embd must be 2*n_embd iff separate_out");
    if (c.hidden % c.heads) return fail(ZETT_E_INVALID, "hidden %d not divisible by heads %d", c.hidden, c.heads);
    const int d = c.hidden / c.heads;
    if (d < 8 || d > 512 || (d & (d - 1))) return fail(ZETT_E_INVALID, "head_dim %d unsupported (need a power of two in [8,512])", d);
    const int kq = precision == ZETT_PREC_F32 ? 32 : 64;
    for (int k : {c.n_in_embd, c.hidden, c.intermediate})
        if (k % kq) return fail(ZETT_E_INVALID, "contraction width %d is not a multiple of %d", k, kq);
    if (c.n_embd % 4) return fail(ZETT_E_INVALID, "n_embd must be a multiple of 4");
    if (c.n_extra < 1) return fail(ZETT_E_INVALID, "n_extra must be >= 1 (reference allocates max(hn_n_extra_tokens,1))");
    if (c.pad_token_id < 0) return fail(ZETT_E_INVALID, "pad_token_id is required");
    if (c.embed_lang && c.n_langs <= 0) return fail(ZETT_E_INVALID, "hn_embed_lang_id needs n_langs");
    return 0;
}

struct WorkspaceSizes {
    int64_t chunk_tokens;
    size_t table, x0, f32_rows, lo_rows, big, stats;
    size_t total() const { return table + x0 + 3 * f32_rows + 3 * lo_rows + big + stats; }
};

static int64_t pair_keys(const zett_config& c, int seq) {
    return ((int64_t)c.original_vocab_size + c.n_extra + 1) * (int64_t)(seq + (c.embed_lang ? 1 : 0));
}

static size_t plan_i32_bytes(const zett_config& c, int64_t N, int seq) {
    const int64_t V = (int64_t)c.original_vocab_size + c.n_extra;
    const int64_t max_tok = N * (int64_t)(seq + (c.embed_lang ? 1 : 0));
    const int64_t K = pair_keys(c, seq);
    const size_t scan_scratch = 2 * ((size_t)std::max<int64_t>(std::max<int64_t>(N, V), K) / SCAN_CHUNK + 2) + 1;
    return ((size_t)N + (N + 1) + 3 + V + (V + 1) + V + 7 * (size_t)max_tok + 2 * (size_t)K + 2 + scan_scratch) * 4;
}

static int64_t chunk_token_cap(const zett_config& c, size_t es) {
    const size_t wide = (size_t)std::max(c.intermediate, 3 * c.hidden);
    const size_t per_token = (size_t)c.n_in_embd * es + 3 * (size_t)c.hidden * 4 + 3 * (size_t)c.hidden * es + wide * es + 24;
    return std::max<int64_t>(131072, (int64_t)(((size_t)12 << 30) / per_token));
}

static WorkspaceSizes workspace_sizes(const zett_config& c, size_t es, int seq, int64_t Ttot, int64_t D, int64_t cap) {
    const int lam = c.embed_lang ? 1 : 0;
    WorkspaceSizes w{};
    if (cap <= 0) cap = chunk_token_cap(c, es);
    w.chunk_tokens = std::max<int64_t>(std::min<int64_t>(cap, std::max<int64_t>(Ttot, D)), seq + lam);
    const size_t MC = (size_t)w.chunk_tokens, MCS = MC + 768;
    const size_t wide = (size_t)std::max(c.intermediate, 3 * c.hidden);
    w.table = (size_t)D * c.hidden * 4;
    w.x0 = MCS * c.n_in_embd * es;
    w.f32_rows = MCS * c.hidden * 4;
    w.lo_rows = MCS * c.hidden * es;
    w.big = MCS * wide * es;
    w.stats = 2 * MCS * 2 * sizeof(float);
    return w;
}
// ... 83 lines not shown

template <typename T>
int do_forward(zett_hypernet* h, const int32_t* sfm, int64_t N, int seq, const void* src, int src_dtype, const zett_dest* dest,
               int64_t v_src, int lang_index, float* out_in, float* out_out, float* out_bias, hipStream_t st);
template <typename T>
int do_table_rows(zett_hypernet* h, const int32_t* id_list, int first, int count, const void* src, int src_dtype, void* table_out, float* stats_out, hipStream_t st);

}

extern "C" {

const char* zett_last_error(void) { return g_err.c_str(); }
int zett_abi_version(void) { return ZETT_ABI_VERSION; }

int zett_create(const zett_config* cfg, int device, int precision, zett_hypernet** out) {
    if (!cfg || !out) return fail(ZETT_E_INVALID, "null argument");
    if (precision != ZETT_PREC_BF16 && precision != ZETT_PREC_F32 && precision != ZETT_PREC_F16) return fail(ZETT_E_INVALID, "unknown precision %d", precision);
    if (int rc = validate_config(*cfg, precision)) return rc;
    int ndev = 0;
    HIP_TRY(hipGetDeviceCount(&ndev));
    if (device < 0 || device >= ndev) return fail(ZETT_E_INVALID, "device %d out of range (%d visible)", device, ndev);
    ZETT_ON_DEVICE(device);
    auto* h = new zett_hypernet();
    h->cfg = *cfg;
    h->device = device;
    h->precision = precision;
    if (hipMalloc((void**)&h->range_word, 64) != hipSuccess || hipHostMalloc((void**)&h->range_host, 64, hipHostMallocDefault) != hipSuccess ||
        hipMemset(h->range_word, 0, 64) != hipSuccess) {
        if (h->range_word) (void)hipFree(h->range_word);
        if (h->range_host) (void)hipHostFree(h->range_host);
        delete h;
        return fail(ZETT_E_HIP, "allocation of the range word failed");
    }
    *out = h;
    return 0;
}

int zett_destroy(zett_hypernet* h) {
    if (!h) return 0;
    ::zett::DeviceScope _scope(h->device);
    for (auto& kv : h->w) {
        if (kv.second.f32) (void)hipFree(kv.second.f32);
        if (kv.second.lo && kv.second.lo != (void*)kv.second.f32) (void)hipFree(kv.second.lo);
    }
    for (void* p : h->owned) (void)hipFree(p);
    for (DevBuf* b : {&h->table, &h->x0, &h->yf, &h->yt, &h->big, &h->pre, &h->ctx, &h->cf, &h->ct, &h->lnstats, &h->lnparts, &h->dest_word, &h->dest_stage[0], &h->dest_stage[1], &h->dest_sink})
        b->release();
    for (zett_hypernet::PlanSlot* psp : {&h->plan[0], &h->plan[1], &h->table_plan}) {
        zett_hypernet::PlanSlot& ps = *psp;
        ps.i32.release(); ps.u8.release();
        if (ps.host) (void)hipHostFree(ps.host);
        if (ps.done) (void)hipEventDestroy(ps.done);
        if (ps.released) (void)hipEventDestroy(ps.released);
    }
    if (h->plan_stream) (void)hipStreamDestroy(h->plan_stream);
    if (h->plan_fork) (void)hipEventDestroy(h->plan_fork);
    if (h->range_word) (void)hipFree(h->range_word);
    if (h->range_host) (void)hipHostFree(h->range_host);
    if (h->dest_host) (void)hipHostFree(h->dest_host);
    if (h->dest_checked) (void)hipEventDestroy(h->dest_checked);
    for (hipEvent_t e : h->out_ready) if (e) (void)hipEventDestroy(e);
    for (hipEvent_t e : h->lane_ev) if (e) (void)hipEventDestroy(e);
    if (h->lane_stream) (void)hipStreamDestroy(h->lane_stream);
    for (hipEvent_t e : h->ev) (void)hipEventDestroy(e);
    delete h;
    return 0;
}

int zett_load_weight(zett_hypernet* h, const char* name, const void* data, int dtype, const int64_t* shape, int ndim) {
    if (!h || !name || !data || !shape || ndim < 1) return fail(ZETT_E_INVALID, "null argument");
    if (h->finalized) return fail(ZETT_E_STATE, "weights are frozen after zett_finalize");
    std::map<std::string, std::vector<int64_t>> exp;
    expected_shapes(h->cfg, exp);
    const std::string n(name);
    auto it = exp.find(n);
    if (it == exp.end()) return 0;
    std::vector<int64_t> got(shape, shape + ndim);
    if (got != it->second) {
        std::string a, b;
        for (auto v : got) a += std::to_string(v) + ",";
        for (auto v : it->second) b += std::to_string(v) + ",";
        return fail(ZETT_E_INVALID, "%s: shape [%s] does not match the config's [%s]", name, a.c_str(), b.c_str());
    }
    ZETT_ON_DEVICE(h->device);
    size_t numel = 1;
    for (auto v : got) numel *= (size_t)v;
    Tensor& t = h->w[n];
    if (t.f32) { (void)hipFree(t.f32); t.f32 = nullptr; }
    t.shape = got;
    t.numel = numel;
    HIP_TRY(hipMalloc((void**)&t.f32, numel * 4));
    if (dtype == ZETT_F32) {
        HIP_TRY(hipMemcpy(t.f32, data, numel * 4, hipMemcpyDefault));
    } else if (dtype == ZETT_F16 || dtype == ZETT_BF16) {
        void* stage = nullptr;
        HIP_TRY(hipMalloc(&stage, numel * 2));
        hipError_t e = hipMemcpy(stage, data, numel * 2, hipMemcpyDefault);
        if (e == hipSuccess) {
            const int blocks = (int)std::min<size_t>((numel + 255) / 256, 65535);
            if (dtype == ZETT_F16) hipLaunchKernelGGL(convert_to_f32_kernel<1>, dim3(blocks), dim3(256), 0, 0, stage, t.f32, numel);
            else hipLaunchKernelGGL(convert_to_f32_kernel<2>, dim3(blocks), dim3(256), 0, 0, stage, t.f32, numel);
            e = hipDeviceSynchronize();
        }
        (void)hipFree(stage);
        if (e != hipSuccess) return fail(ZETT_E_HIP, "upload of %s failed: %s", name, hipGetErrorString(e));
    } else {
        return fail(ZETT_E_INVALID, "unknown dtype %d", dtype);
    }
    return 0;
}

int zett_finalize(zett_hypernet* h) {
    if (!h) return fail(ZETT_E_INVALID, "null handle");
    if (h->finalized) return 0;
    ZETT_ON_DEVICE(h->device);
    std::map<std::string, std::vector<int64_t>> exp;
    expected_shapes(h->cfg, exp);
    for (auto& kv : exp)
        if (!h->w.count(kv.first)) return fail(ZETT_E_STATE, "missing weight: %s", kv.first.c_str());
    const zett_config& c = h->cfg;
    const size_t es = elt_size(h->precision);
    for (auto& kv : h->w) {
        Tensor& t = kv.second;
        if (!is_gemm_weight(kv.first)) continue;
        if (h->precision == ZETT_PREC_F32) { t.lo = t.f32; continue; }
        HIP_TRY(hipMalloc(&t.lo, t.numel * 2));
        const int blocks = (int)std::min<size_t>((t.numel / 4 + 255) / 256 + 1, 65535);
        if (h->precision == ZETT_PREC_F16)
            hipLaunchKernelGGL(convert_f32_to_lo_kernel<f16_t>, dim3(blocks), dim3(256), 0, 0, t.f32, (f16_t*)t.lo, t.numel, h->range_word);
        else
            hipLaunchKernelGGL(convert_f32_to_lo_kernel<bf16_t>, dim3(blocks), dim3(256), 0, 0, t.f32, (bf16_t*)t.lo, t.numel, h->range_word);
    }
    HIP_TRY(hipDeviceSynchronize());
    const size_t H = c.hidden;
    for (int l = 0; l < c.layers; ++l) {
        const std::string p = "model.encoder.layer." + std::to_string(l) + ".attention.self.";
        void* wq = nullptr; float* bq = nullptr;
        HIP_TRY(hipMalloc(&wq, 3 * H * H * es));
        HIP_TRY(hipMalloc((void**)&bq, 3 * H * 4));
        h->owned.push_back(wq); h->owned.push_back(bq);
        int k = 0;
        for (const char* q : {"query", "key", "value"}) {
            Tensor& tw = h->w[p + q + ".weight"];
            Tensor& tb = h->w[p + q + ".bias"];
            HIP_TRY(hipMemcpy((char*)wq + (size_t)k * H * H * es, tw.lo, H * H * es, hipMemcpyDeviceToDevice));
            HIP_TRY(hipMemcpy(bq + (size_t)k * H, tb.f32, H * 4, hipMemcpyDeviceToDevice));
            ++k;
        }
        h->qkv_w.push_back(wq);
        h->qkv_b.push_back(bq);
    }
    if (h->precision != ZETT_PREC_F32 && c.hidden % 128 == 0) {
        auto fold = [&](const float* w32, size_t N, size_t K, const float* gamma, const float* beta, const float* bias,
                        zett_hypernet::Folded& f) -> int {
            HIP_TRY(hipMalloc(&f.w, N * K * es));
            HIP_TRY(hipMalloc((void**)&f.c, N * 4));
            HIP_TRY(hipMalloc((void**)&f.b, N * 4));
            h->owned.push_back(f.w); h->owned.push_back(f.c); h->owned.push_back(f.b);
            if (h->precision == ZETT_PREC_F16)
                hipLaunchKernelGGL(fold_weight_kernel<f16_t>, dim3((unsigned)N), dim3(256), 0, 0, w32, (int)K, gamma, beta, bias, (f16_t*)f.w, f.c, f.b, h->range_word);
            else
                hipLaunchKernelGGL(fold_weight_kernel<bf16_t>, dim3((unsigned)N), dim3(256), 0, 0, w32, (int)K, gamma, beta, bias, (bf16_t*)f.w, f.c, f.b, h->range_word);
            return 0;
        };
        h->fold_qkv.resize(c.layers); h->fold_up.resize(c.layers);
        float* tmp = nullptr;
        HIP_TRY(hipMalloc((void**)&tmp, 3 * H * H * 4));
        for (int l = 0; l < c.layers; ++l) {
            const std::string lp = "model.encoder.layer." + std::to_string(l) + ".";
            if (int rc = fold(h->w[lp + "intermediate.dense.weight"].f32, c.intermediate, H, h->w[lp + "attention.output.LayerNorm.weight"].f32,
                              h->w[lp + "attention.output.LayerNorm.bias"].f32, h->w[lp + "intermediate.dense.bias"].f32, h->fold_up[l])) return rc;
            if (l == 0) continue;
            const std::string pp = "model.encoder.layer." + std::to_string(l - 1) + ".output.LayerNorm.";
            int k = 0;
            for (const char* q : {"query", "key", "value"}) {
                HIP_TRY(hipMemcpy(tmp + (size_t)k * H * H, h->w[lp + "attention.self." + q + ".weight"].f32, H * H * 4, hipMemcpyDeviceToDevice));
                ++k;
            }
            if (int rc = fold(tmp, 3 * H, H, h->w[pp + "weight"].f32, h->w[pp + "bias"].f32, h->qkv_b[l], h->fold_qkv[l])) return rc;
        }
        if (!(c.single_head && c.separate_out)) {
            const size_t w0 = c.single_head ? c.n_in_embd : c.n_embd;
            if (int rc = fold(h->w["output_projection.1.weight"].f32, w0, H, h->w["output_projection.0.ln.weight"].f32,
                              h->w["output_projection.0.ln.bias"].f32, h->w["output_projection.1.bias"].f32, h->fold_head_in)) return rc;
            if (c.separate_out && !c.single_head)
                if (int rc = fold(h->w["output_projection_out.1.weight"].f32, c.n_embd, H, h->w["output_projection_out.0.ln.weight"].f32,
                                  h->w["output_projection_out.0.ln.bias"].f32, h->w["output_projection_out.1.bias"].f32, h->fold_head_out)) return rc;
            std::vector<float> ones(w0, 1.0f), zeros(w0, 0.0f);
            HIP_TRY(hipMalloc((void**)&h->head_one, w0 * 4));
            HIP_TRY(hipMalloc((void**)&h->head_zero, w0 * 4));
            h->owned.push_back(h->head_one); h->owned.push_back(h->head_zero);
            HIP_TRY(hipMemcpy(h->head_one, ones.data(), w0 * 4, hipMemcpyHostToDevice));
            HIP_TRY(hipMemcpy(h->head_zero, zeros.data(), w0 * 4, hipMemcpyHostToDevice));
        }
        HIP_TRY(hipDeviceSynchronize());
        (void)hipFree(tmp);
    }
    HIP_TRY(hipMemcpy(h->range_host, h->range_word, 4, hipMemcpyDeviceToHost));
    if (h->range_host[0] & ZETT_RANGE_WEIGHT)
        return fail(ZETT_E_RANGE, "a GEMM weight (or a LayerNorm-folded weight W*gamma) exceeds the half range (|w| > 65504 or not finite): "
                                  "this checkpoint needs ZETT_PREC_BF16 or ZETT_PREC_F32");
    if (c.rescale) {
        const size_t w0 = c.single_head ? c.n_in_embd : c.n_embd;
        HIP_TRY(hipMalloc((void**)&h->head_scale, w0 * 4));
        HIP_TRY(hipMalloc((void**)&h->head_shift, w0 * 4));
        h->owned.push_back(h->head_scale); h->owned.push_back(h->head_shift);
        HIP_TRY(hipMemcpy(h->head_scale, h->w["scaler.w"].f32, c.n_embd * 4, hipMemcpyDeviceToDevice));
        HIP_TRY(hipMemcpy(h->head_shift, h->w["scaler.b"].f32, c.n_embd * 4, hipMemcpyDeviceToDevice));
        if (c.single_head && c.separate_out) {
            HIP_TRY(hipMemcpy(h->head_scale + c.n_embd, h->w["out_scaler.w"].f32, c.n_embd * 4, hipMemcpyDeviceToDevice));
            HIP_TRY(hipMemcpy(h->head_shift + c.n_embd, h->w["out_scaler.b"].f32, c.n_embd * 4, hipMemcpyDeviceToDevice));
        }
    }
    if (h->precision != ZETT_PREC_F32) {
        for (auto& kv : h->w) {
            Tensor& t = kv.second;
            if (is_gemm_weight(kv.first) && t.f32) { (void)hipFree(t.f32); t.f32 = nullptr; }
        }
    }
    h->finalized = true;
    return 0;
}

int zett_set_option(zett_hypernet* h, const char* key, int64_t value) {
    if (!h || !key) return fail(ZETT_E_INVALID, "null argument");
    const std::string k(key);
    if (k == "max_chunk_tokens") {
        if (value < 1024) return fail(ZETT_E_INVALID, "max_chunk_tokens must be >= 1024");
        h->max_chunk_tokens = value;
    } else if (k == "time_gemm") {
        h->time_gemm = value != 0;
    } else if (k == "cls_only_last_layer") {
        h->cls_only_last = value != 0;
    } else if (k == "pair_dedupe") {
        h->pair_dedupe = value != 0;
    } else if (k == "residual_lo") {
        if (value < 0 || value > 2) return fail(ZETT_E_INVALID, "residual_lo must be 0 (fp32 residual stream), 1 (16-bit stream in f16 mode) or 2 (in bf16 mode too)");
        h->residual_lo = (int)value;
    } else if (k == "concurrent_lanes") {
        if (value < 0 || value > 2) return fail(ZETT_E_INVALID, "concurrent_lanes must be 0 (never), 1 (auto) or 2 (whenever a call is one chunk of >= 512 rows)");
        h->concurrent_lanes = (int)value;
    } else if (k == "attention_fast") {
        h->attention_fast = value != 0;
    } else if (k == "ln_fold") {
        if (value < 0 || value > 2) return fail(ZETT_E_INVALID, "ln_fold must be 0 (off), 1 (encoder and output heads) or 2 (encoder only: A/B)");
        h->ln_fold = (int)value;
    } else if (k == "gemm_tail_split") {
        if (value < 0 || value > 3) return fail(ZETT_E_INVALID, "gemm_tail_split must be 0 (never), 1 (auto), 2 (cut every gemm4d launch in the middle) or 3 (128x256 tiles only)");
        h->gemm_tail_split = (int)value;
    } else if (k == "attention_pack") {
        h->attention_pack = value != 0;
    } else if (k == "ln_rows8") {
        h->ln_rows8 = value != 0;
    } else if (k == "table_lo") {
        h->table_lo = value != 0;
    } else if (k == "gemm_group") {
        if (value < 0 || value > 64) return fail(ZETT_E_INVALID, "gemm_group must be 0 (default: 4) .. 64");
        h->gemm_group = (int)value;
    } else if (k == "gemm_tile_order") {
        if (value < 0 || value > 1) return fail(ZETT_E_INVALID, "gemm_tile_order must be 0 or 1");
        h->gemm_tile_order = (int)value;
    } else if (k == "gemm4d_min_k") {
        if (value < 64) return fail(ZETT_E_INVALID, "gemm4d_min_k must be >= 64");
        h->gemm4d_min_k = (int)value;
    } else if (k == "range_accumulate") {
        h->range_accumulate = value != 0;
    } else if (k == "gemm_variant") {
        if (value != 0 && value != 1 && value != 2 && value != 3 && value != 7 && value != 8)
            return fail(ZETT_E_INVALID, "gemm_variant must be 0 (auto), 1 (128x128), 2 (256x256 register-staged), 3 (384x256), 7 (256x256 four-wave direct-to-LDS) or 8 (7 with the generic epilogue drain)");
        h->gemm_variant = (int)value;
    } else {
        return fail(ZETT_E_INVALID, "unknown option %s", key);
    }
    return 0;
}

int zett_workspace_bytes(const zett_hypernet* h, int64_t n_rows, int32_t seq, int64_t* out_bytes) {
    if (!h || !out_bytes) return fail(ZETT_E_INVALID, "null argument");
    if (n_rows < 0 || seq < 1) return fail(ZETT_E_INVALID, "bad surface-form shape [%lld, %d]", (long long)n_rows, seq);
    const zett_config& c = h->cfg;
    const int64_t V = (int64_t)c.original_vocab_size + c.n_extra;
    const int64_t max_tok = n_rows * (int64_t)(seq + (c.embed_lang ? 1 : 0));
    const WorkspaceSizes w = workspace_sizes(c, elt_size(h->precision), seq, max_tok, std::min<int64_t>(V, max_tok), h->max_chunk_tokens);
    const size_t parts = c.hidden % 128 == 0 ? (size_t)(c.hidden / 128) * ((size_t)w.chunk_tokens + 768) * 8 : 0;
    *out_bytes = (int64_t)(w.total() + parts + plan_i32_bytes(c, n_rows, seq) + (size_t)n_rows + (size_t)max_tok);
    return 0;
}

int zett_get_stats(const zett_hypernet* h, zett_stats* out) {
    if (!h || !out) return fail(ZETT_E_INVALID, "null argument");
    *out = h->stats;
    return 0;
}

int zett_stream_wait_output(zett_hypernet* h, int which, void* stream) {
    if (!h) return fail(ZETT_E_INVALID, "null handle");
    if (which != ZETT_OUT_IN && which != ZETT_OUT_BIAS) return fail(ZETT_E_INVALID, "which must be ZETT_OUT_IN or ZETT_OUT_BIAS");
    if (!h->out_recorded) return fail(ZETT_E_STATE, "no forward has run on this handle");
    ZETT_ON_DEVICE(h->device);
    HIP_TRY(hipStreamWaitEvent((hipStream_t)stream, h->out_ready[which], 0));
    return 0;
}

int zett_get_gemm_log(const zett_hypernet* h, zett_gemm_record* out, int64_t capacity, int64_t* count) {
    if (!h || !count || capacity < 0 || (capacity > 0 && !out)) return fail(ZETT_E_INVALID, "null argument");
    *count = (int64_t)h->gemm_log.size();
    for (int64_t i = 0; i < capacity && i < *count; ++i) out[i] = h->gemm_log[(size_t)i];
    return 0;
}

int zett_check_range(zett_hypernet* h, void* stream, int32_t* flags) {
    if (!h) return fail(ZETT_E_INVALID, "null handle");
    ZETT_ON_DEVICE(h->device);
    hipStream_t st = (hipStream_t)stream;
    HIP_TRY(hipMemcpyAsync(h->range_host, h->range_word, 4, hipMemcpyDeviceToHost, st));
    HIP_TRY(hipStreamSynchronize(st));
    const int32_t w = h->range_host[0];
    if (h->range_accumulate && w) HIP_TRY(hipMemsetAsync(h->range_word, 0, 4, st));
    if (flags) *flags = w;
    if (!w) return 0;
    return fail(ZETT_E_RANGE, "the last forward left the range of its arithmetic:%s%s%s%s (precision %s)",
                (w & ZETT_RANGE_SOURCE) ? " in_scaler(source_embeddings) beyond the half range;" : "",
                (w & ZETT_RANGE_ACTIVATION) ? " a 16-bit activation (Q/K/V, FFN intermediate or the operand copy of the residual sum) beyond the half range;" : "",
                (w & ZETT_RANGE_OUTPUT) ? " non-finite predicted embeddings;" : "",
                (w & ZETT_RANGE_DEST) ? " a finite value beyond the range of an f16 destination (stored as inf);" : "",
                h->precision == ZETT_PREC_F16 ? "f16: re-run with ZETT_PREC_BF16" : h->precision == ZETT_PREC_BF16 ? "bf16" : "f32");
}

int zett_partition_workspace_bytes(int64_t n_rows, int32_t n_ids, int64_t* out_bytes) {
    if (!out_bytes || n_rows < 0 || n_ids < 1) return fail(ZETT_E_INVALID, "bad argument");
    *out_bytes = (int64_t)partition_workspace_bytes(n_rows, n_ids);
    return 0;
}

int zett_partition_rows(const int32_t* surface_forms, int64_t n_rows, int32_t seq, int32_t pad_id, int32_t n_ids, int32_t world,
                        const int32_t* caps, int32_t* perm_out, void* workspace, int64_t workspace_bytes, int32_t device, void* stream) {
    if (n_rows < 0 || seq < 1 || n_ids < 1) return fail(ZETT_E_INVALID, "bad surface-form shape [%lld, %d] / id range %d", (long long)n_rows, seq, n_ids);
    if (world < 1 || world > PART_MAX_RANKS) return fail(ZETT_E_INVALID, "zett_partition_rows handles 1..%d ranks (one node), got %d", PART_MAX_RANKS, world);
    if (n_rows == 0) return 0;
    if (!surface_forms || !caps || !perm_out || !workspace) return fail(ZETT_E_INVALID, "null argument");
    if (n_rows >= (int64_t)0x7fffffff) return fail(ZETT_E_INVALID, "too many rows for one call");
    int64_t total = 0;
    for (int r = 0; r < world; ++r) { if (caps[r] < 0) return fail(ZETT_E_INVALID, "negative capacity"); total += caps[r]; }
    if (total != n_rows) return fail(ZETT_E_INVALID, "the ranks' capacities sum to %lld, the matrix has %lld rows", (long long)total, (long long)n_rows);
    if ((size_t)workspace_bytes < partition_workspace_bytes(n_rows, n_ids)) return fail(ZETT_E_INVALID, "workspace too small (zett_partition_workspace_bytes)");
    ZETT_ON_DEVICE(device);
    hipStream_t st = (hipStream_t)stream;
    const size_t have_bytes = ((size_t)(n_ids + 3) / 4) * 4 + 64;
    uint32_t* have = (uint32_t*)workspace;
    PartCaps caps_arg = {};
    for (int r = 0; r < world; ++r) caps_arg.v[r] = caps[r];
    HIP_TRY(hipMemsetAsync(have, 0, have_bytes, st));
    const size_t lds_have = ((size_t)(n_ids + 3) / 4) * 4;
    if (lds_have <= 150 * 1024) {
        static bool attr_set[64] = {};
        if (device >= 64 || !attr_set[device]) {
            HIP_TRY(hipFuncSetAttribute((const void*)partition_rows_kernel<true>, hipFuncAttributeMaxDynamicSharedMemorySize, 150 * 1024));
            if (device < 64) attr_set[device] = true;
        }
        hipLaunchKernelGGL(partition_rows_kernel<true>, dim3(1), dim3(PART_THREADS), lds_have, st, surface_forms, n_rows, (int)seq, (int)pad_id, (int)n_ids,
                           (int)world, caps_arg, have, perm_out);
    } else {
        hipLaunchKernelGGL(partition_rows_kernel<false>, dim3(1), dim3(PART_THREADS), 0, st, surface_forms, n_rows, (int)seq, (int)pad_id, (int)n_ids,
                           (int)world, caps_arg, have, perm_out);
    }
    HIP_TRY(hipGetLastError());
    return 0;
}

int zett_scatter_rows(const void* src, void* dst, const int64_t* order, int64_t n_rows, int64_t row_bytes, int32_t device, void* stream) {
    if (n_rows < 0 || row_bytes < 1) return fail(ZETT_E_INVALID, "bad shape");
    if (n_rows == 0) return 0;
    if (!src || !dst || !order) return fail(ZETT_E_INVALID, "null argument");
    if (row_bytes != 4 && row_bytes % 16 != 0) return fail(ZETT_E_INVALID, "row_bytes must be 4 or a multiple of 16, got %lld", (long long)row_bytes);
    if (((uintptr_t)src | (uintptr_t)dst) % (row_bytes == 4 ? 4 : 16)) return fail(ZETT_E_INVALID, "misaligned buffer");
    ZETT_ON_DEVICE(device);
    hipStream_t st = (hipStream_t)stream;
    if (row_bytes == 4)
        hipLaunchKernelGGL(scatter_words_kernel, dim3((unsigned)((n_rows + 255) / 256)), dim3(256), 0, st, (const uint32_t*)src, (uint32_t*)dst, order, n_rows);
    else
        hipLaunchKernelGGL(scatter_rows_kernel, dim3((unsigned)std::min<int64_t>(n_rows, 65535 * 16)), dim3(256), 0, st, (const unsigned char*)src, (unsigned char*)dst,
                           order, n_rows, row_bytes);
    HIP_TRY(hipGetLastError());
    return 0;
}

int zett_forward_prepare(zett_hypernet* h, const int32_t* surface_forms, int64_t n_rows, int32_t seq, void* input_stream) {
    if (!h) return fail(ZETT_E_INVALID, "null handle");
    if (!h->finalized) return fail(ZETT_E_STATE, "zett_finalize has not been called");
    const zett_config& c = h->cfg;
    if (n_rows < 0 || seq < 1) return fail(ZETT_E_INVALID, "bad surface-form shape [%lld, %d]", (long long)n_rows, seq);
    if (n_rows == 0) return 0;
    if (!surface_forms) return fail(ZETT_E_INVALID, "null tensor argument");
    if (n_rows * (int64_t)(seq + 1) >= (int64_t)0x7fffffff) return fail(ZETT_E_INVALID, "too many positions for one call");
    (void)c;
    ZETT_ON_DEVICE(h->device);
    if (!h->plan_stream) {
        int least = 0, greatest = 0;
        HIP_TRY(hipDeviceGetStreamPriorityRange(&least, &greatest));
        HIP_TRY(hipStreamCreateWithPriority(&h->plan_stream, hipStreamNonBlocking, greatest));
    }
    if (!h->plan_fork) HIP_TRY(hipEventCreateWithFlags(&h->plan_fork, hipEventDisableTiming));
    zett_hypernet::PlanSlot& ps = h->plan[h->plan_cur ^ 1];
    if (ps.pending) HIP_TRY(hipEventSynchronize(ps.done));
    HIP_TRY(hipEventRecord(h->plan_fork, (hipStream_t)input_stream));
    HIP_TRY(hipStreamWaitEvent(h->plan_stream, h->plan_fork, 0));
    if (ps.released) HIP_TRY(hipStreamWaitEvent(h->plan_stream, ps.released, 0));
    if (int rc = enqueue_plan(h, ps, surface_forms, n_rows, seq, h->plan_stream)) return rc;
// ... 200 lines not shown
    if (variant == 3 && (N % 256 != 0 || (long)((M + 383) / 384) * 384 > a_rows_readable || e.scale || e.shift || e.residual || e.range_final)) variant = 2;
    if (h->gemm_variant == 0 && variant == 2 && !is_f32 && K >= h->gemm4d_min_k) variant = 7;
    if ((variant == 7 || variant == 8) && is_f32) variant = 2;
    const bool wide_ok = N % 8 == 0 && (!e.out_lo || e.ld_lo % 8 == 0) && e.ld_f32 % 4 == 0 && (!e.residual || e.ld_res % 4 == 0) &&
                         (e.split_col >= N || e.split_col % 8 == 0);
    if (variant != 1 && !wide_ok) variant = 1;
    if (e.residual && (e.scale || e.shift)) variant = 1;
    if (e.stats_part || e.fold_stats) variant = 7;
        return variant;
    }


    void gemm(const T* A, int lda, const T* Wp, int ldw, int M, int N, int K, const GemmEpilogue<T>& e) {
        if (rc || M <= 0) return;
        GemmArgs<T> g{A, lda, Wp, ldw, M, N, K, e};
        g.tile_order = h->gemm_tile_order;
        g.group = h->gemm_group;
        g.row0 = h->gemm_tail_split == 1 ? -1 : h->gemm_tail_split == 2 ? ((M / 2 + 255) / 256) * 256 : h->gemm_tail_split == 3 ? -2 : 0;
        const double fl = 2.0 * (double)M * (double)N * (double)K;
        hipEvent_t e0 = nullptr, e1 = nullptr;
        if (h->time_gemm) {
            while (h->ev.size() < h->ev_used + 2) {
                hipEvent_t ev;
                if (hipEventCreate(&ev) != hipSuccess) { rc = fail(ZETT_E_HIP, "hipEventCreate failed"); return; }
                h->ev.push_back(ev);
            }
            e0 = h->ev[h->ev_used++];
            e1 = h->ev[h->ev_used++];
            h->ev_flops.push_back(fl);
            h->ev_shape.push_back({M, N, K, 0});
            (void)hipEventRecord(e0, st);
        }
        const int variant = variant_for(M, N, K, e);
        if (h->time_gemm && !h->ev_shape.empty()) h->ev_shape.back()[3] = variant;
        {
            zett_gemm_record r{};
            r.m = M; r.n = N; r.k = K; r.variant = variant;
            r.epilogue = (e.out_lo ? 1 : 0) | ((e.out_f32 || e.out_f32_b) ? 2 : 0) | (e.residual ? 4 : 0) | ((e.scale || e.shift) ? 8 : 0) |
                         (e.stats_part ? 16 : 0) | (e.fold_stats ? 32 : 0) | (e.residual_lo ? 64 : 0) | (e.act << 8) |
                         (e.dst ? 1024 : 0) | (staged_dst ? 2048 : 0);
            r.flops = fl;
            const double mn = (double)M * (double)N;
            const double dst_es = e.dst_dtype == ZETT_F32 ? 4.0 : 2.0;
            r.bytes = ((double)M + (double)N) * (double)K * sizeof(T) + (e.out_lo ? mn * sizeof(T) : 0.0) + ((e.out_f32 || e.out_f32_b) ? mn * 4.0 : 0.0) +
                      (e.dst ? mn * dst_es : 0.0) +
                      (e.residual ? mn * 4.0 : 0.0) + (e.residual_lo ? mn * sizeof(T) : 0.0) + (e.stats_part ? (double)M * (N / 128) * 8.0 : 0.0) + ((e.fold_stats || e.res_stats) ? (double)M * 8.0 : 0.0);
            h->gemm_log.push_back(r);
        }
        const hipError_t err = launch_gemm_variant(variant, g, st);
        if (h->time_gemm) (void)hipEventRecord(e1, st);
        if (err != hipSuccess) { rc = fail(ZETT_E_HIP, "gemm launch failed: %s", hipGetErrorString(err)); return; }
        h->stats.executed_flops += fl;
        h->stats.gemm_launches += 1;
    }

    struct DestOut { void* p; const int64_t* rows; int64_t ld; int dtype; };

    void head_gemm(const T* A, const T* Wp, int M, int N, int K, const GemmEpilogue<T>& e, const DestOut* d, const DestOut* d_b, int split) {
        if (rc || M <= 0) return;
        if (!d) { gemm(A, K, Wp, K, M, N, K, e); return; }
        GemmEpilogue<T> ed = e;
        ed.out_f32 = nullptr; ed.out_f32_b = nullptr; ed.ld_f32 = N;
        ed.dst = d->p; ed.dst_rows = d->rows; ed.ld_dst = d->ld; ed.dst_dtype = d->dtype;
        const GemmArgs<T> probe{A, K, Wp, K, M, N, K, ed};
        if (!d_b && variant_for(M, N, K, ed) == 7 && gemm_4d_dst_mode(probe) >= 0) { gemm(A, K, Wp, K, M, N, K, ed); return; }
        DevBuf& stage_buf = h->dest_stage[stage_lane];
        if (int r = stage_buf.reserve((size_t)M * (size_t)N * sizeof(float))) { rc = r; return; }
        float* S = stage_buf.as<float>();
        GemmEpilogue<T> es = e;
        es.out_f32 = S; es.ld_f32 = N;
        if (d_b) es.out_f32_b = S + split;
        staged_dst = true;
        gemm(A, K, Wp, K, M, N, K, es);
        staged_dst = false;
        dest_store(S, N, *d, M, d_b ? split : N);
        if (d_b) dest_store(S + split, N, *d_b, M, N - split);
    }

    void dest_store(const float* S, int64_t ld_s, const DestOut& d, int rows, int cols) {
        if (rc || rows <= 0) return;
        const bool vec = cols % 4 == 0 && ld_s % 4 == 0 && d.ld % 4 == 0 && (uintptr_t)S % 16 == 0 && (uintptr_t)d.p % (d.dtype == ZETT_F32 ? 16 : 8) == 0;
        const dim3 grid((unsigned)std::min<int64_t>(rows, 65535 * 16));
#define ZETT_DEST_STORE(OT) do { if (vec) hipLaunchKernelGGL((dest_store_rows_kernel<OT, true>), grid, dim3(256), 0, st, S, ld_s, (OT*)d.p, d.ld, d.rows, (int64_t)rows, cols, h->range_word); \
                                 else hipLaunchKernelGGL((dest_store_rows_kernel<OT, false>), grid, dim3(256), 0, st, S, ld_s, (OT*)d.p, d.ld, d.rows, (int64_t)rows, cols, h->range_word); } while (0)
        if (d.dtype == ZETT_F16) ZETT_DEST_STORE(f16_t);
        else if (d.dtype == ZETT_BF16) ZETT_DEST_STORE(bf16_t);
        else ZETT_DEST_STORE(float);
#undef ZETT_DEST_STORE
        check("dest_store");
    }

    template <typename BT>
    void readout_dst(const float* in, int rows, const float* gamma, const float* beta, float eps, float* of, T* ol, const LnReadout& readout) {
        const int H = h->cfg.hidden;
        if constexpr (sizeof(T) == 2) {
            const int tpr8 = h->ln_rows8 ? ln_rows8_tpr(H) : 0;
            if (tpr8) {
                const dim3 grid8((rows + 256 / tpr8 - 1) / (256 / tpr8));
                if (tpr8 == 32) hipLaunchKernelGGL((layernorm_rows8_kernel<T, false, 32, true, BT>), grid8, dim3(256), 0, st, in, H, rows, H, gamma, beta, eps, of, ol, (float*)nullptr, (float*)nullptr, LnEmbed{}, 0, readout);
                else hipLaunchKernelGGL((layernorm_rows8_kernel<T, false, 64, true, BT>), grid8, dim3(256), 0, st, in, H, rows, H, gamma, beta, eps, of, ol, (float*)nullptr, (float*)nullptr, LnEmbed{}, 0, readout);
                check("readout");
                return;
            }
        }
        if (H <= 2048) hipLaunchKernelGGL((layernorm_rows_kernel<T, false, 64, true, BT>), dim3((rows + 3) / 4), dim3(256), 0, st, in, H, rows, H, gamma, beta, eps, of, ol, (float*)nullptr, (float*)nullptr, LnEmbed{}, 0, readout);
        else hipLaunchKernelGGL((layernorm_rows_kernel<T, false, 256, true, BT>), dim3(rows), dim3(256), 0, st, in, H, rows, H, gamma, beta, eps, of, ol, (float*)nullptr, (float*)nullptr, LnEmbed{}, 0, readout);
        check("readout");
    }

    void check(const char* what) {
        if (rc) return;
        hipError_t e = hipGetLastError();
        if (e != hipSuccess) rc = fail(ZETT_E_HIP, "%s launch failed: %s", what, hipGetErrorString(e));
    }

    void layernorm(const float* in, int rows, const float* gamma, const float* beta, float eps, float* of, T* ol, float* stats = nullptr,
                   LnReadout readout = LnReadout{}, const T* in_lo = nullptr, int bias_dtype = -1) {
        if (rc || rows <= 0) return;
        readout.in_lo = in_lo;
        if (bias_dtype >= 0 && readout.out_bias) {
            if (bias_dtype == ZETT_F16) readout_dst<f16_t>(in, rows, gamma, beta, eps, of, ol, readout);
            else if (bias_dtype == ZETT_BF16) readout_dst<bf16_t>(in, rows, gamma, beta, eps, of, ol, readout);
            else readout_dst<float>(in, rows, gamma, beta, eps, of, ol, readout);
            return;
        }
        const int H = h->cfg.hidden;
        if constexpr (sizeof(T) == 2) {
            const int tpr8 = h->ln_rows8 ? ln_rows8_tpr(H) : 0;
            if (tpr8) {
                const dim3 grid8((rows + 256 / tpr8 - 1) / (256 / tpr8));
#define ZETT_LN8_LAUNCH(TPR, RO) hipLaunchKernelGGL((layernorm_rows8_kernel<T, false, TPR, RO>), grid8, dim3(256), 0, st, in, H, rows, H, gamma, beta, eps, of, ol, stats, (float*)nullptr, LnEmbed{}, 0, readout)
                if (readout.out_bias) { if (tpr8 == 32) ZETT_LN8_LAUNCH(32, true); else ZETT_LN8_LAUNCH(64, true); }
                else { if (tpr8 == 32) ZETT_LN8_LAUNCH(32, false); else ZETT_LN8_LAUNCH(64, false); }
#undef ZETT_LN8_LAUNCH
                check("layernorm");
                return;
            }
        }
        const dim3 grid = H <= 2048 ? dim3((rows + 3) / 4) : dim3(rows);
#define ZETT_LN_LAUNCH(TPR, RO) hipLaunchKernelGGL((layernorm_rows_kernel<T, false, TPR, RO>), grid, dim3(256), 0, st, in, H, rows, H, gamma, beta, eps, of, ol, stats, (float*)nullptr, LnEmbed{}, 0, readout)
        if (readout.out_bias) { if (H <= 2048) ZETT_LN_LAUNCH(64, true); else ZETT_LN_LAUNCH(256, true); }
        else { if (H <= 2048) ZETT_LN_LAUNCH(64, false); else ZETT_LN_LAUNCH(256, false); }
#undef ZETT_LN_LAUNCH
        check("layernorm");
    }

    void ln_stats(const float2* parts, int ld_part, int rows, float eps, float* stats) {
        if (rc || rows <= 0) return;
        hipLaunchKernelGGL(ln_stats_kernel, dim3((rows + 63) / 64), dim3(64), 0, st, parts, h->cfg.hidden / 128, ld_part, rows,
                           h->cfg.hidden, eps, stats);
        check("ln_stats");
    }

    void projector(const std::string& p, const T* x_lo, const float* x_f32, int rows, T* big, float* pre, float* of, T* ol,
                   float2* fold_parts = nullptr, int ld_part = 0, float* fold_stats = nullptr) {
        const zett_config& c = h->cfg;
        GemmEpilogue<T> e1 = epi();
        e1.bias = Wf(p + "dense1.bias"); e1.act = ACT_GELU_TANH; e1.out_lo = big; e1.ld_lo = c.intermediate;
        gemm(x_lo, c.hidden, Wlo(p + "dense1.weight"), c.hidden, rows, c.intermediate, c.hidden, e1);
        GemmEpilogue<T> e2 = epi();
        e2.bias = Wf(p + "dense2.bias"); e2.act = ACT_GELU_TANH; e2.residual = x_f32; e2.ld_res = c.hidden;
        e2.ld_f32 = c.hidden;
        if (fold_parts) { e2.out_lo = ol; e2.ld_lo = c.hidden; e2.stats_part = fold_parts; e2.ld_part = ld_part; }
        else e2.out_f32 = pre;
        gemm(big, c.intermediate, Wlo(p + "dense2.weight"), c.intermediate, rows, c.hidden, c.intermediate, e2);
        if (fold_parts) ln_stats(fold_parts, ld_part, rows, c.ln_eps_projector, fold_stats);
        else layernorm(pre, rows, Wf(p + "ln.weight"), Wf(p + "ln.bias"), c.ln_eps_projector, of, ol);
    }
};

template <typename T, int SD>
void launch_gather(hipStream_t st, const int32_t* id_list, int s0, int m, const void* src, const zett_config& c,
                   const float* fallback, const float* sw, const float* sb, T* out, int32_t* range_flag) {
    hipLaunchKernelGGL((gather_src_kernel<T, SD>), dim3(m), dim3(256), 0, st, id_list, s0, m, src, c.n_in_embd,
                       c.original_vocab_size, fallback, sw, sb, out, range_flag);
}

template <typename T>
void table_phase(Runner<T>& R, const int32_t* id_list, int first, int count, const void* src, int src_dtype, int64_t MC, size_t MCS,
                 T* X0, float* Zf, T* Zt, T* BIG, float* PRE, float2* PARTS, bool table_lo, T* tbl16, float* tblst, float* tbl32) {
    zett_hypernet* h = R.h;
    const zett_config& c = h->cfg;
    const int H = c.hidden, EIN = c.n_in_embd;
    hipStream_t st = R.st;
    const float* in_w = c.rescale ? R.Wf("in_scaler.w") : nullptr;
    const float* in_b = c.rescale ? R.Wf("in_scaler.b") : nullptr;
    for (int s0 = first; s0 < first + count && !R.rc; s0 += (int)MC) {
        const int m = (int)std::min<int64_t>(MC, first + count - s0);
        const float* fb = R.Wf("fallback_embeddings.weight");
        if (src_dtype == ZETT_F32) launch_gather<T, 0>(st, id_list, s0, m, src, c, fb, in_w, in_b, X0, h->range_word);
        else if (src_dtype == ZETT_F16) launch_gather<T, 1>(st, id_list, s0, m, src, c, fb, in_w, in_b, X0, h->range_word);
        else launch_gather<T, 2>(st, id_list, s0, m, src, c, fb, in_w, in_b, X0, h->range_word);
        R.check("gather_src");
        GemmEpilogue<T> e0 = R.epi();
        e0.bias = R.Wf("input_projection.0.bias"); e0.out_f32 = Zf; e0.ld_f32 = H; e0.out_lo = Zt; e0.ld_lo = H;
        R.gemm(X0, EIN, R.Wlo("input_projection.0.weight"), EIN, m, H, EIN, e0);
        if (table_lo) R.projector("input_projection.1.", Zt, Zf, m, BIG, PRE, nullptr, tbl16 + (size_t)s0 * H, PARTS, (int)MCS, tblst + 2 * (size_t)s0);
        else R.projector("input_projection.1.", Zt, Zf, m, BIG, PRE, tbl32 + (size_t)s0 * H, nullptr);
    }
}

template <typename T>
bool folded_table_mode(const zett_hypernet* h) {
    const zett_config& c = h->cfg;
    const int H = c.hidden;
    const bool fold = h->ln_fold && !std::is_same<T, float>::value && h->gemm_variant == 0 && H % 128 == 0 && H >= 512 && (int)h->fold_up.size() == c.layers;
    const bool lo_stream = fold && c.layers >= 1 && sizeof(T) == 2 && (h->residual_lo == 2 || (h->residual_lo == 1 && std::is_same<T, f16_t>::value));
    return lo_stream && h->table_lo != 0;
}

template <typename T>
int do_table_rows(zett_hypernet* h, const int32_t* id_list, int first, int count, const void* src, int src_dtype, void* table_out, float* stats_out, hipStream_t st) {
    const zett_config& c = h->cfg;
    if (!folded_table_mode<T>(h))
        return fail(ZETT_E_INVALID, "zett_table_rows needs the folded 16-bit table: f16 arithmetic with the LayerNorm fold, the 16-bit residual stream and table_lo on");
    const WorkspaceSizes ws = workspace_sizes(c, sizeof(T), 1, count, count, h->max_chunk_tokens);
    const int64_t MC = ws.chunk_tokens;
    const size_t MCS = (size_t)MC + 768;
    if (int rc = h->x0.reserve(ws.x0)) return rc;
    if (int rc = h->yf.reserve(ws.f32_rows)) return rc;
    if (int rc = h->yt.reserve(ws.lo_rows)) return rc;
    if (int rc = h->big.reserve(ws.big)) return rc;
    if (int rc = h->pre.reserve(ws.f32_rows)) return rc;
    if (int rc = h->lnparts.reserve((size_t)(c.hidden / 128) * MCS * sizeof(float2))) return rc;
    Runner<T> R{h, st};
    R.a_rows_readable = (long)MCS;
    struct NoTiming { zett_hypernet* h; int saved; ~NoTiming() { h->time_gemm = saved; } } no_timing{h, h->time_gemm};
    h->time_gemm = 0;
    table_phase<T>(R, id_list, first, count, src, src_dtype, MC, MCS, h->x0.as<T>(), h->yf.as<float>(), h->yt.as<T>(), h->big.as<T>(), h->pre.as<float>(),
                   h->lnparts.as<float2>(), true, (T*)table_out, stats_out, nullptr);
    return R.rc;
}

template <typename T>
int do_forward(zett_hypernet* h, const int32_t* sfm, int64_t N, int seq, const void* src, int src_dtype, const zett_dest* dest,
               int64_t v_src, int lang_index, float* out_in, float* out_out, float* out_bias, hipStream_t st) {
    (void)v_src;
    const zett_config& c = h->cfg;
    const int H = c.hidden, I = c.intermediate, E = c.n_embd, EIN = c.n_in_embd;
    const int lam = c.embed_lang ? 1 : 0;
    const int V = c.original_vocab_size + c.n_extra;
    const int64_t max_tok = N * (int64_t)(seq + lam);
    h->stats = zett_stats{};
    h->stats.rows = N;
    h->ev_used = 0;
    h->ev_flops.clear();
    h->ev_shape.clear();
    h->gemm_log.clear();

    zett_hypernet::PlanSlot& ps = h->plan[h->plan_cur ^ 1];
    if (ps.pending && ps.sfm == sfm && ps.n_rows == N && ps.seq == seq && ps.pair_plan == plan_layout(h, ps, N, seq).pair_plan &&
        ps.ext_id_slot == h->ext.id_slot) {
        HIP_TRY(hipStreamWaitEvent(st, ps.done, 0));
    } else {
        if (ps.pending) HIP_TRY(hipEventSynchronize(ps.done));
        if (ps.released) HIP_TRY(hipStreamWaitEvent(st, ps.released, 0));
        if (int rc = enqueue_plan(h, ps, sfm, N, seq, st)) return rc;
    }
    ps.pending = false;
    h->plan_cur ^= 1;
    struct SlotGuard {
        zett_hypernet* h; zett_hypernet::PlanSlot* ps; hipStream_t st; bool lane_forked = false;
        ~SlotGuard() {
            if (lane_forked && h->lane_stream && h->lane_ev[3]) {
                (void)hipEventRecord(h->lane_ev[3], h->lane_stream);
                (void)hipStreamWaitEvent(st, h->lane_ev[3], 0);
            }
            if (ps->released) (void)hipEventRecord(ps->released, st);
        }
    } slot_guard{h, &ps, st};
    const PlanLayout PL = plan_layout(h, ps, N, seq);
    const PlanArrays& p = PL.p;
    const bool pair_plan = PL.pair_plan;
    if (!h->range_accumulate) HIP_TRY(hipMemsetAsync(h->range_word, 0, 4, st));
    for (hipEvent_t& e : h->out_ready)
        if (!e) HIP_TRY(hipEventCreateWithFlags(&e, hipEventDisableTiming));
    const bool dest_check = dest && dest->rows;
    if (dest_check) {
        if (int rc = h->dest_word.reserve(4)) return rc;
        if (!h->dest_host) HIP_TRY(hipHostMalloc((void**)&h->dest_host, 4, hipHostMallocDefault));
        if (!h->dest_checked) HIP_TRY(hipEventCreateWithFlags(&h->dest_checked, hipEventDisableTiming));
        HIP_TRY(hipMemsetAsync(h->dest_word.p, 0, 4, st));
        hipLaunchKernelGGL(dest_rows_check_kernel, dim3((unsigned)((N + 255) / 256)), dim3(256), 0, st, dest->rows, N, dest->n_dest_rows, h->dest_word.as<int32_t>());
        HIP_TRY(hipGetLastError());
        HIP_TRY(hipMemcpyAsync(h->dest_host, h->dest_word.p, 4, hipMemcpyDeviceToHost, st));
        HIP_TRY(hipEventRecord(h->dest_checked, st));
    }
    HIP_TRY(hipEventSynchronize(ps.done));
    int32_t* hoff = ps.host;
    if (hoff[N + 2] != 0)
        return fail(ZETT_E_INDEX, "surface-form row %d holds an id outside [0, %d) (original_vocab_size %d + %d fallback rows)",
                    hoff[N + 2] - 1, V, c.original_vocab_size, c.n_extra);
    if (dest_check) {
        HIP_TRY(hipEventSynchronize(h->dest_checked));
        if (h->dest_host[0] != 0)
            return fail(ZETT_E_INDEX, "destination row map: rows[%d] is outside the destination's %lld rows", h->dest_host[0] - 1, (long long)dest->n_dest_rows);
    }
    const int64_t Ttot = hoff[N];
    const int D = hoff[N + 1];
    h->stats.packed_tokens = Ttot;
    h->stats.distinct_ids = D;
    h->stats.distinct_positions = Ttot;

    const WorkspaceSizes ws = workspace_sizes(c, sizeof(T), seq, Ttot, D, h->max_chunk_tokens);
    const int64_t MC = ws.chunk_tokens;
    const size_t MCS = (size_t)MC + 768;
    if (int rc = h->table.reserve(ws.table)) return rc;
    if (int rc = h->x0.reserve(ws.x0)) return rc;
    if (int rc = h->yf.reserve(ws.f32_rows)) return rc;
    if (int rc = h->yt.reserve(ws.lo_rows)) return rc;
    if (int rc = h->big.reserve(ws.big)) return rc;
    if (int rc = h->pre.reserve(ws.f32_rows)) return rc;
    if (int rc = h->ctx.reserve(ws.lo_rows)) return rc;
    if (int rc = h->cf.reserve(ws.f32_rows)) return rc;
    if (int rc = h->ct.reserve(ws.lo_rows)) return rc;
    if (int rc = h->lnstats.reserve(ws.stats)) return rc;
    const bool fold = h->ln_fold && !std::is_same<T, float>::value && h->gemm_variant == 0 && H % 128 == 0 && H >= 512 &&
                      (int)h->fold_up.size() == c.layers;
    const bool lo_stream = fold && c.layers >= 1 && sizeof(T) == 2 &&
                           (h->residual_lo == 2 || (h->residual_lo == 1 && std::is_same<T, f16_t>::value));
    const size_t ws_parts = fold ? (size_t)(H / 128) * MCS * sizeof(float2) : 0;
    if (int rc = h->lnparts.reserve(ws_parts)) return rc;
    float2* PARTS = h->lnparts.as<float2>();
    float* TBL = h->table.as<float>();
    const bool table_lo = lo_stream && h->table_lo != 0;
    const bool ext_table = h->ext.table != nullptr;
    if (ext_table && !table_lo)
        return fail(ZETT_E_INVALID, "zett_forward_table needs the folded 16-bit table: f16 arithmetic with the LayerNorm fold, the 16-bit residual stream and table_lo on");
    T* TBL16 = ext_table ? (T*)const_cast<void*>(h->ext.table) : (T*)h->table.as<float>();
    float* TBLST = ext_table ? const_cast<float*>(h->ext.stats) : (float*)((char*)h->table.as<float>() + (((size_t)D * H * sizeof(T) + 15) / 16) * 16);
    T* X0 = h->x0.as<T>();
    float* Zf = h->yf.as<float>();
    T* Zt = h->yt.as<T>();
    T* BIG = h->big.as<T>();
    float* PRE = h->pre.as<float>();
    T* CTX = h->ctx.as<T>();
    float* Cf = h->cf.as<float>();
    T* Ct = h->ct.as<T>();
    float* STa = h->lnstats.as<float>();
    float* STb = STa + 2 * MCS;

    Runner<T> R{h, st};
    R.a_rows_readable = (long)MCS;

    if (!ext_table)
        table_phase<T>(R, p.id_list, 0, D, src, src_dtype, MC, MCS, X0, Zf, Zt, BIG, PRE, PARTS, table_lo, TBL16, TBLST, TBL);
    if (R.rc) return R.rc;

    const float* lang_vec = lam ? R.Wf("lang_embeddings.weight") + (size_t)lang_index * H : nullptr;
    const float scaling = 1.0f / std::sqrt((float)(H / c.heads));
// ... 29 lines not shown
        float* hs_sum = Zf;
        float* hs_stats = STb;
        const float* hs_gamma = R.Wf("model.embeddings.LayerNorm.weight");
        const float* hs_beta = R.Wf("model.embeddings.LayerNorm.bias");
        auto embed_ln = [&](const LnEmbed& e, int n, int t0, T* lo, float* stats, float* sum) {
            if constexpr (sizeof(T) == 2) {
                const int tpr8 = h->ln_rows8 ? ln_rows8_tpr(H) : 0;
                if (tpr8) {
                    const dim3 grid8((n + 256 / tpr8 - 1) / (256 / tpr8));
                    if (tpr8 == 32)
                        hipLaunchKernelGGL((layernorm_rows8_kernel<T, true, 32, false>), grid8, dim3(256), 0, st, (const float*)nullptr, H, n, H,
                                           hs_gamma, hs_beta, c.ln_eps_encoder, (float*)nullptr, lo, stats, sum, e, t0, LnReadout{});
                    else
                        hipLaunchKernelGGL((layernorm_rows8_kernel<T, true, 64, false>), grid8, dim3(256), 0, st, (const float*)nullptr, H, n, H,
                                           hs_gamma, hs_beta, c.ln_eps_encoder, (float*)nullptr, lo, stats, sum, e, t0, LnReadout{});
                    R.check("embed_layernorm");
                    return;
                }
            }
            if (H <= 2048)
                hipLaunchKernelGGL((layernorm_rows_kernel<T, true, 64>), dim3((n + 3) / 4), dim3(256), 0, st, (const float*)nullptr, H, n, H,
                                   hs_gamma, hs_beta, c.ln_eps_encoder, (float*)nullptr, lo, stats, sum, e, t0, LnReadout{});
            else
                hipLaunchKernelGGL((layernorm_rows_kernel<T, true, 256>), dim3(n), dim3(256), 0, st, (const float*)nullptr, H, n, H,
                                   hs_gamma, hs_beta, c.ln_eps_encoder, (float*)nullptr, lo, stats, sum, e, t0, LnReadout{});
            R.check("embed_layernorm");
        };
        const int P = pair_plan ? hoff[N + 3] : 0;
        const bool pairs = pair_plan && rows == N && P > 0 && (int64_t)P * 100 <= (int64_t)m * 85;
        int32_t* brow_pair = p.tok_pkey;
        if (pairs) {
            LnEmbed pe = emb;
            pe.tok_slot = p.pair_tslot; pe.tok_pos = p.pair_pos; pe.tok_row = nullptr;
            embed_ln(pe, P, 0, Zt, hs_stats, lo_stream ? (float*)nullptr : hs_sum);
            hipLaunchKernelGGL(pair_rows_kernel, dim3((m + 255) / 256), dim3(256), 0, st, m, tok0, r0, rows, p, brow_pair);
            R.check("pair_rows");
            h->stats.distinct_positions = P;
        } else {
            embed_ln(emb, m, tok0, Zt, hs_stats, lo_stream ? (float*)nullptr : hs_sum);
        }

        int zrows = m;
        bool raw = false;
        auto other = [&](float* b) { return b == Zf ? PRE : Zf; };
        auto other_stats = [&](float* b) { return b == STa ? STb : STa; };
        for (int l = 0; l < c.layers && !R.rc; ++l) {
            const std::string lp = "model.encoder.layer." + std::to_string(l) + ".";
            const bool last = l == c.layers - 1;
            const bool cls_only = h->cls_only_last && last;
            const T* wqkv = raw ? (const T*)h->fold_qkv[l].w : (const T*)h->qkv_w[l];
            const float* bqkv = raw ? h->fold_qkv[l].b : h->qkv_b[l];
            const float* cqkv = raw ? h->fold_qkv[l].c : nullptr;
            const int64_t waves = attention_waves(rows, H, h->attention_pack != 0).total;
            const int att_flags = (h->attention_fast ? 2 : 0) | (h->attention_pack ? 4 : 0);
            if (!cls_only) {
                const bool by_pair = pairs && l == 0;
                GemmEpilogue<T> eq = R.epi();
                eq.bias = bqkv; eq.out_lo = BIG; eq.ld_lo = 3 * H;
                if (raw) { eq.fold_stats = hs_stats; eq.fold_c = cqkv; }
                R.gemm(Zt, H, wqkv, H, by_pair ? P : m, 3 * H, H, eq);
                hipLaunchKernelGGL((attention_rows_kernel<T>), dim3((unsigned)((waves + 3) / 4)), dim3(256), 0, st,
                                   (const T*)BIG, (size_t)3 * H, (const T*)BIG + H, (const T*)BIG + 2 * H, (size_t)3 * H,
                                   H, H / c.heads, p.row_offset, p.row_uniform, p.tok_key, r0, rows, tok0, scaling, 0 | att_flags,
                                   by_pair ? (const int32_t*)p.tok_pair : (const int32_t*)nullptr, CTX);
                R.check("attention");
            } else {
                T* KV = BIG;
                T* Q = BIG + (size_t)m * 2 * H;
                GemmEpilogue<T> ekv = R.epi();
                ekv.bias = bqkv + H; ekv.out_lo = KV; ekv.ld_lo = 2 * H;
                if (raw) { ekv.fold_stats = hs_stats; ekv.fold_c = cqkv + H; }
                R.gemm(Zt, H, wqkv + (size_t)H * H, H, m, 2 * H, H, ekv);
                GemmEpilogue<T> eq = R.epi();
                eq.bias = bqkv; eq.out_lo = Q; eq.ld_lo = H;
                if (raw) { eq.fold_stats = hs_stats; eq.fold_c = cqkv; }
                R.gemm(Zt, H, wqkv, H, rows, H, H, eq);
                hipLaunchKernelGGL((attention_rows_kernel<T>), dim3((unsigned)((waves + 3) / 4)), dim3(256), 0, st,
                                   (const T*)Q, (size_t)H, (const T*)KV, (const T*)KV + H, (size_t)2 * H,
                                   H, H / c.heads, p.row_offset, p.row_uniform, p.tok_key, r0, rows, tok0, scaling, 1 | att_flags,
                                   (const int32_t*)nullptr, CTX);
                R.check("attention(position 0)");
                zrows = rows;
            }
            float* s1 = other(hs_sum);
            float* st1 = other_stats(hs_stats);
            GemmEpilogue<T> eo = R.epi();
            eo.bias = R.Wf(lp + "attention.output.dense.bias");
            if (pairs && l == 0) eo.res_index = brow_pair;
            if (lo_stream) {
                eo.residual_lo = Zt; eo.ld_res_lo = H;
                if (raw) { eo.res_stats = hs_stats; eo.res_gamma = hs_gamma; eo.res_beta = hs_beta; }
                eo.out_lo = Ct; eo.ld_lo = H; eo.stats_part = PARTS; eo.ld_part = (int)ld_parts;
            } else {
                eo.residual = hs_sum; eo.ld_res = H;
                eo.res_stats = hs_stats; eo.res_gamma = hs_gamma; eo.res_beta = hs_beta;
                eo.out_f32 = s1; eo.ld_f32 = H;
                if (fold) { eo.out_lo = Zt; eo.ld_lo = H; eo.stats_part = PARTS; eo.ld_part = (int)ld_parts; }
            }
            R.gemm(CTX, H, R.Wlo(lp + "attention.output.dense.weight"), H, zrows, H, H, eo);
            const float* g1 = R.Wf(lp + "attention.output.LayerNorm.weight");
            const float* b1 = R.Wf(lp + "attention.output.LayerNorm.bias");
            const T* mid = lo_stream ? Ct : Zt;
            GemmEpilogue<T> ei = R.epi();
            ei.act = ACT_GELU_ERF; ei.out_lo = BIG; ei.ld_lo = I;
            if (fold) {
                R.ln_stats(PARTS, (int)ld_parts, zrows, c.ln_eps_encoder, st1);
                ei.bias = h->fold_up[l].b; ei.fold_stats = st1; ei.fold_c = h->fold_up[l].c;
                R.gemm(mid, H, (const T*)h->fold_up[l].w, H, zrows, I, H, ei);
            } else {
                R.layernorm(s1, zrows, g1, b1, c.ln_eps_encoder, nullptr, Zt, st1);
                ei.bias = R.Wf(lp + "intermediate.dense.bias");
                R.gemm(Zt, H, R.Wlo(lp + "intermediate.dense.weight"), H, zrows, I, H, ei);
            }
            float* s2 = other(s1);
            float* st2 = other_stats(st1);
            GemmEpilogue<T> ef = R.epi();
            ef.bias = R.Wf(lp + "output.dense.bias");
            if (lo_stream) {
                ef.residual_lo = Ct; ef.ld_res_lo = H; ef.res_stats = st1; ef.res_gamma = g1; ef.res_beta = b1;
                ef.out_lo = Zt; ef.ld_lo = H; ef.stats_part = PARTS; ef.ld_part = (int)ld_parts;
            } else {
                ef.residual = s1; ef.ld_res = H;
                ef.res_stats = st1; ef.res_gamma = g1; ef.res_beta = b1;
                ef.out_f32 = s2; ef.ld_f32 = H;
                if (fold && !last) { ef.out_lo = Zt; ef.ld_lo = H; ef.stats_part = PARTS; ef.ld_part = (int)ld_parts; }
            }
            R.gemm(BIG, I, R.Wlo(lp + "output.dense.weight"), I, zrows, H, I, ef);
            hs_gamma = R.Wf(lp + "output.LayerNorm.weight");
            hs_beta = R.Wf(lp + "output.LayerNorm.bias");
            hs_sum = s2; hs_stats = st2;
            if (!last) {
                if (fold) { R.ln_stats(PARTS, (int)ld_parts, zrows, c.ln_eps_encoder, st2); raw = true; }
                else R.layernorm(s2, zrows, hs_gamma, hs_beta, c.ln_eps_encoder, nullptr, Zt, st2);
            }
        }
        if (R.rc) return R.rc;

        float* bias_out = out_bias ? out_bias + r0 : nullptr;
        const int64_t* bias_rows = nullptr;
        int bias_dtype = -1;
        if (dest && dest->bias) {
            const size_t bes = dest->bias_dtype == ZETT_F32 ? 4 : 2;
            bias_rows = dest->rows ? dest->rows + r0 : nullptr;
            bias_out = (float*)((char*)dest->bias + (dest->rows ? 0 : (size_t)r0 * bes));
            bias_dtype = dest->bias_dtype;
        } else if (dest) {
            if (int rc = h->dest_sink.reserve((size_t)N * sizeof(float))) return rc;
            bias_out = h->dest_sink.as<float>() + r0;
        }
        LnReadout ro{c.predict_bias ? R.Wf("bias_projection.weight") : (const float*)nullptr,
                     c.predict_bias ? R.Wf("bias_projection.bias") : (const float*)nullptr, bias_out};
        ro.bias_rows = bias_rows;
        ro.range_flag = h->range_word;
        R.layernorm(hs_sum, rows, hs_gamma, hs_beta, c.ln_eps_encoder, Cf, Ct, nullptr, ro,
                    lo_stream ? (const T*)Zt : (const T*)nullptr, bias_dtype);
        R.check("readout");
        if (!R.rc) {
            if (ev_mode == 2) HIP_TRY(hipEventRecord(h->lane_ev[1], st));
            if (ev_mode == 3) HIP_TRY(hipStreamWaitEvent(st, h->lane_ev[1], 0));
            if (ev_mode == 1 || ev_mode == 3) HIP_TRY(hipEventRecord(h->out_ready[ZETT_OUT_BIAS], st));
        }

        const bool fold_heads = fold && h->ln_fold == 1 && h->fold_head_in.w != nullptr;
        {
            if (fold_heads) R.projector("output_projection.0.", Ct, Cf, rows, BIG, PRE, nullptr, CTX, PARTS, (int)ld_parts, STa);
            else R.projector("output_projection.0.", Ct, Cf, rows, BIG, PRE, nullptr, CTX);
            GemmEpilogue<T> e = R.epi();
            e.bias = fold_heads ? h->fold_head_in.b : R.Wf("output_projection.1.bias");
            e.scale = c.rescale ? h->head_scale : (fold_heads ? h->head_one : nullptr);
            e.shift = c.rescale ? h->head_shift : (fold_heads ? h->head_zero : nullptr);
            if (fold_heads) { e.fold_stats = STa; e.fold_c = h->fold_head_in.c; }
            e.ld_f32 = E; e.range_final = 1;
            const int width = c.single_head ? EIN : E;
            const bool split = c.single_head && c.separate_out;
            if (!dest) {
                e.out_f32 = out_in + (size_t)r0 * E;
                if (split) { e.split_col = E; e.out_f32_b = out_out + (size_t)r0 * E; }
            } else if (split) {
                e.split_col = E;
            }
            const T* w1 = fold_heads ? (const T*)h->fold_head_in.w : R.Wlo("output_projection.1.weight");
            if (dest) {
                const typename Runner<T>::DestOut din = dest_out(dest->in, dest->ld_in, r0), dout = dest_out(dest->out, dest->ld_out, r0);
                R.head_gemm(CTX, w1, rows, width, H, e, &din, split ? &dout : nullptr, E);
            } else {
                R.gemm(CTX, H, w1, H, rows, width, H, e);
            }
            if (!R.rc) {
                if (ev_mode == 2) HIP_TRY(hipEventRecord(h->lane_ev[2], st));
                if (ev_mode == 3) HIP_TRY(hipStreamWaitEvent(st, h->lane_ev[2], 0));
                if (ev_mode == 1 || ev_mode == 3) HIP_TRY(hipEventRecord(h->out_ready[ZETT_OUT_IN], st));
            }
        }
        if (c.separate_out && !c.single_head) {
            if (fold_heads) R.projector("output_projection_out.0.", Ct, Cf, rows, BIG, PRE, nullptr, CTX, PARTS, (int)ld_parts, STa);
            else R.projector("output_projection_out.0.", Ct, Cf, rows, BIG, PRE, nullptr, CTX);
            GemmEpilogue<T> e = R.epi();
            e.bias = fold_heads ? h->fold_head_out.b : R.Wf("output_projection_out.1.bias");
            e.scale = c.rescale ? R.Wf("out_scaler.w") : (fold_heads ? h->head_one : nullptr);
            e.shift = c.rescale ? R.Wf("out_scaler.b") : (fold_heads ? h->head_zero : nullptr);
            if (fold_heads) { e.fold_stats = STa; e.fold_c = h->fold_head_out.c; }
            e.ld_f32 = E; e.range_final = 1;
            const T* w2 = fold_heads ? (const T*)h->fold_head_out.w : R.Wlo("output_projection_out.1.weight");
            if (dest) {
                const typename Runner<T>::DestOut dout = dest_out(dest->out, dest->ld_out, r0);
                R.head_gemm(CTX, w2, rows, E, H, e, &dout, nullptr, E);
            } else {
                e.out_f32 = out_out + (size_t)r0 * E;
                R.gemm(CTX, H, w2, H, rows, E, H, e);
            }
        }
        return R.rc;
    };
    bool two_lanes = false;
    if (h->concurrent_lanes && Ttot <= MC && N >= 512) {
        const int Pn = pair_plan ? hoff[N + 3] : 0;
        const bool pairs_taken = pair_plan && Pn > 0 && (int64_t)Pn * 100 <= Ttot * 85;
        const double r = (double)((Ttot + 255) / 256) * (double)((H + 255) / 256) / 256.0;
        two_lanes = h->concurrent_lanes == 2 ||
                    (!pairs_taken && !h->time_gemm && H >= 1024 && r < 4.0 && (std::ceil(r) - r) / std::ceil(r) > 0.08);
    }
    if (two_lanes) {
        if (!h->lane_stream) HIP_TRY(hipStreamCreateWithFlags(&h->lane_stream, hipStreamNonBlocking));
        for (hipEvent_t& e : h->lane_ev)
            if (!e) HIP_TRY(hipEventCreateWithFlags(&e, hipEventDisableTiming));
        int64_t ra = ((N / 2 + 128) / 256) * 256;
        ra = std::min<int64_t>(std::max<int64_t>(ra, 256), N - 1);
        const size_t off1 = (size_t)(hoff[ra] - hoff[0]) + 384;
        HIP_TRY(hipEventRecord(h->lane_ev[0], st));
        HIP_TRY(hipStreamWaitEvent(h->lane_stream, h->lane_ev[0], 0));
        slot_guard.lane_forked = true;
        if (int rc = run_chunk(ra, N, Lane{h->lane_stream, off1}, 2)) return rc;
        if (int rc = run_chunk(0, ra, Lane{st, 0}, 3)) return rc;
    } else {
        int64_t r0 = 0;
        while (r0 < N) {
            int64_t r1 = r0 + 1;
            while (r1 < N && (int64_t)hoff[r1 + 1] - hoff[r0] <= MC) ++r1;
            if (int rc = run_chunk(r0, r1, Lane{st, 0}, r1 == N ? 1 : 0)) return rc;
            r0 = r1;
        }
    }
    R.st = st;
    if (R.rc) return R.rc;
    if (slot_guard.lane_forked) {
        HIP_TRY(hipEventRecord(h->lane_ev[3], h->lane_stream));
        HIP_TRY(hipStreamWaitEvent(st, h->lane_ev[3], 0));
        slot_guard.lane_forked = false;
    }
    h->out_recorded = true;

    if (h->time_gemm) {
        HIP_TRY(hipStreamSynchronize(st));
        double ms = 0.0, fl = 0.0;
        for (size_t i = 0; i + 1 < h->ev_used; i += 2) {
            float t = 0.f;
            if (hipEventElapsedTime(&t, h->ev[i], h->ev[i + 1]) == hipSuccess) { ms += t; fl += h->ev_flops[i / 2]; }
        }
        h->stats.gemm_ms = ms;
        h->stats.gemm_flops_timed = fl;
        for (size_t i = 0; i + 1 < h->ev_used && i / 2 < h->gemm_log.size(); i += 2) {
            float t = 0.f;
            if (hipEventElapsedTime(&t, h->ev[i], h->ev[i + 1]) == hipSuccess) h->gemm_log[i / 2].ms = t;
        }
        if (getenv("ZETT_GEMM_LOG")) {
            for (size_t i = 0; i + 1 < h->ev_used; i += 2) {
                float t = 0.f;
                (void)hipEventElapsedTime(&t, h->ev[i], h->ev[i + 1]);
                const auto& sh = h->ev_shape[i / 2];
                fprintf(stderr, "[zett gemm] M=%6d N=%6d K=%5d tile=%s %8.3f ms %7.1f TF\n", sh[0], sh[1], sh[2],
                        sh[3] == 7 ? "4d " : sh[3] == 8 ? "4dg" : sh[3] == 3 ? "384" : sh[3] == 2 ? "8r " : "128", t, h->ev_flops[i / 2] / (t * 1e9));
            }
        }
    }
    return 0;
}

}
```

Before: 619,100.

## Fold final encoder LayerNorm into output projector dense1 and use 16-bit residual

Stops materializing the final encoder LayerNorm output before the output projector. A new readout_stats kernel computes the per-row LN stats from the partial sums and does the bias readout. The LN is folded into a precomputed dense1 weight, and dense2's residual is rebuilt from the 16-bit stream with an in-epilogue LN affine. The LN16 GEMM epilogue gains a tanh-GELU variant, and an optional (off by default) 16-bit residual path is added for the input projector. This removes a full LayerNorm pass and its fp32/16-bit writes, at the cost of extra folded weights and some precision risk from folding.

```diff
diff --git a/zett_amd/csrc/gemm.hip.h b/zett_amd/csrc/gemm.hip.h
--- a/zett_amd/csrc/gemm.hip.h
+++ b/zett_amd/csrc/gemm.hip.h
@@ -83,6 +83,11 @@
 __device__ __forceinline__ float ln_affine(float x, float mean, float rstd, float g, float b) {
 #pragma clang fp contract(off)
     return __builtin_fmaf((x - mean) * rstd, g, b);
+}
+
+__device__ __forceinline__ float epi_add(float v, float res) {
+#pragma clang fp contract(off)
+    return v + res;
 }
 
 template <int ACT>
diff --git a/zett_amd/csrc/gemm4d.hip.h b/zett_amd/csrc/gemm4d.hip.h
--- a/zett_amd/csrc/gemm4d.hip.h
+++ b/zett_amd/csrc/gemm4d.hip.h
@@ -190,11 +190,11 @@
     constexpr bool LN16K = EPI == G4D_EPI_LN16;
     uint4 res16[LN16K ? 16 : 1];
     const bool res16_early = LN16K && g.epi.res_index == nullptr;
-    auto res16_request = [&](int p, int t) __attribute__((always_inline)) {
+    auto res16_request = [&](int p, int t, int ln) __attribute__((always_inline)) {
         if constexpr (LN16K) {
-            int grow = m0 + wm * GEO::WROWS + p * 64 + t * 4 + (lane >> 4);
+            int grow = m0 + wm * GEO::WROWS + p * 64 + t * 4 + (ln >> 4);
             grow = grow < g.M ? grow : g.M - 1;
-            int gc = n0 + wn * 128 + (lane & 15) * 8;
+            int gc = n0 + wn * 128 + (ln & 15) * 8;
             gc = gc < g.N ? gc : 0;
             res16[t] = *(const uint4*)(g.epi.residual_lo + (size_t)grow * g.epi.ld_res_lo + gc);
         }
@@ -266,14 +266,14 @@
                 if (DMA && moreA && p >= 70 && p < 102 && WV == ((p - 70) & 3)) dma_a(cur, kt + 2, (p - 70) >> 2);
                 if (RD && more && p >= 103 && p <= 110) read_w(nxt, 0, p - 103);
                 if (RD && more && p >= 111 && p <= 125 && (p & 1) == 1) read_a(nxt, 0, (p - 111) >> 1);
-                if constexpr (LN16K) { if (!more && p >= 40 && p < 104 && (p & 3) == 0 && res16_early) res16_request(0, (p - 40) >> 2); }
+                if constexpr (LN16K) { if (!more && p >= 40 && p < 104 && (p & 3) == 0 && res16_early) res16_request(0, (p - 40) >> 2, lane); }
             } else {
                 if (p >= 16 && p <= 22 && (p & 1) == 0) read_a(cur, 1, (p - 16) >> 1);
                 if (moreA && p >= 27 && p < 43 && (WV & 1) == ((p - 27) & 1)) dma_w(cur, kt + 3, (p - 27) >> 1);
                 if (moreA && p >= 43 && p < 51 && (WV & 1) == ((p - 43) & 1)) dma_a(cur, kt + 3, (p - 43) >> 1);
                 if (more && p >= 53 && p <= 60) read_w(nxt, 0, p - 53);
                 if (more && p >= 60 && p <= 63) read_a(nxt, 0, p - 60);
-                if constexpr (LN16K) { if (!more && p >= 24 && p < 56 && (p & 1) == 0 && res16_early) res16_request(0, (p - 24) >> 1); }
+                if constexpr (LN16K) { if (!more && p >= 24 && p < 56 && (p & 1) == 0 && res16_early) res16_request(0, (p - 24) >> 1, lane); }
             }
             if (!M32 || (p & 1)) __builtin_amdgcn_sched_barrier(0);
         }
@@ -352,7 +352,8 @@
         constexpr bool LNP = EPI == G4D_EPI_F32_LN || EPI == G4D_EPI_LO_LN || LN16, FOLD = EPI == G4D_EPI_LO_FOLD || EPI == G4D_EPI_F32_SCALE_FOLD;
         constexpr bool WF32 = EPI != G4D_EPI_LO_LN && !LN16;
         static_assert(!LNP || RES, "a LayerNorm producer is a residual epilogue");
-        static_assert((EPI != G4D_EPI_F32_LN && !LN16) || ACT == ACT_NONE, "the encoder's producer has no activation");
+        static_assert(EPI != G4D_EPI_F32_LN || ACT == ACT_NONE, "the encoder's fp32 producer has no activation");
+        static_assert(!LN16 || ACT == ACT_NONE || ACT == ACT_GELU_TANH, "16-bit stream: the encoder's producer, or a ProjectorBlock's dense2 (tanh-GELU)");
         static_assert(!LN16 || sizeof(T) == 2, "16-bit residual stream");
         constexpr int CPL = (LO || LN16) ? 8 : 4;
         constexpr int LPR = 128 / CPL;
@@ -383,12 +384,13 @@
                 }
             }
         }
-        const bool res_ln = RES && ACT == ACT_NONE && e.res_stats != nullptr;
+        constexpr bool RES_LN = RES && (ACT == ACT_NONE || LN16);
+        const bool res_ln = RES_LN && e.res_stats != nullptr;
         float lg[CPL], lb[CPL];
 #pragma unroll
         for (int c = 0; c < CPL; ++c) { lg[c] = 1.f; lb[c] = 0.f; }
         float2 pst[2] = {make_float2(0.f, 1.f), make_float2(0.f, 1.f)};
-        if constexpr (RES && ACT == ACT_NONE) {
+        if constexpr (RES_LN) {
             if (res_ln) {
                 if (col_ok) {
 #pragma unroll
@@ -454,7 +456,7 @@
                         const size_t rrow = (size_t)__shfl(rix[p], t * RPI + rsub, 64);
                         res16[t] = (grow < g.M && col_ok) ? *(const uint4*)(e.residual_lo + rrow * e.ld_res_lo + gcol) : make_uint4(0u, 0u, 0u, 0u);
                     } else {
-                        res16_request(p, t);
+                        res16_request(p, t, ACT == ACT_GELU_TANH ? lane_e : lane);
                     }
                 }
             }
@@ -488,10 +490,24 @@
             if constexpr (LN16)
                 *(float2*)(region + lane_e * G4D_EPI_STRIDE + 128) = pst[p];
         };
-        auto drain = [&](int p, auto full_c) {
+        auto drain = [&](int p, auto full_c) __attribute__((always_inline)) {
             constexpr bool FULL = decltype(full_c)::value;
             constexpr int GROUP = (LO || RES) ? 4 : 8;
             constexpr int NV = GROUP * CPL;
+            constexpr bool LN16T = LN16 && ACT == ACT_GELU_TANH;
+            constexpr int LN16T_NV = 16;
+            auto res16_values = [&](int t, float (&r8)[8]) __attribute__((always_inline)) {
+                if constexpr (LN16) {
+                    const uint4 x = res16[t];
+                    unpack2_lo<T>(x.x, r8[0], r8[1]); unpack2_lo<T>(x.y, r8[2], r8[3]);
+                    unpack2_lo<T>(x.z, r8[4], r8[5]); unpack2_lo<T>(x.w, r8[6], r8[7]);
+                    if (res_ln) {
+                        const float2 st = *(const float2*)(region + (t * RPI + rsub) * G4D_EPI_STRIDE + 128);
+#pragma unroll
+                        for (int c = 0; c < 8; ++c) r8[c] = ln_affine(r8[c], st.x, st.y, lg[c], lb[c]);
+                    }
+                }
+            };
             float acc_s = 0.f, acc_q = 0.f;
 #pragma unroll
             for (int t0 = 0; t0 < NIT; t0 += GROUP) {
@@ -506,7 +522,8 @@
                     }
 #pragma unroll
                     for (int c = 0; c < CPL; ++c) { bb[u * CPL + c] = bias[c]; ss[u * CPL + c] = sc[c]; hh[u * CPL + c] = sh[c]; rr[u * CPL + c] = 0.f; }
-                    if constexpr (LN16) {
+                    if constexpr (LN16T) {
+                    } else if constexpr (LN16) {
                         const uint4 x = res16[t0 + u];
                         unpack2_lo<T>(x.x, rr[u * 8], rr[u * 8 + 1]); unpack2_lo<T>(x.y, rr[u * 8 + 2], rr[u * 8 + 3]);
                         unpack2_lo<T>(x.z, rr[u * 8 + 4], rr[u * 8 + 5]); unpack2_lo<T>(x.w, rr[u * 8 + 6], rr[u * 8 + 7]);
@@ -545,6 +562,22 @@
                         }
                     }
                 }
+                if constexpr (LN16T) {
+#pragma unroll
+                    for (int hv = 0; hv < NV / LN16T_NV; ++hv) {
+                        typedef float part_t[LN16T_NV];
+                        epi_values<ACT, false, false, LN16T_NV>(*(part_t*)(v + LN16T_NV * hv), *(const part_t*)(bb + LN16T_NV * hv), *(const part_t*)(rr + LN16T_NV * hv),
+                                                                *(const part_t*)(ss + LN16T_NV * hv), *(const part_t*)(hh + LN16T_NV * hv));
+                    }
+                    __builtin_amdgcn_sched_barrier(0);
+#pragma unroll
+                    for (int u = 0; u < GROUP; ++u) {
+                        float r8[8];
+                        res16_values(t0 + u, r8);
+#pragma unroll
+                        for (int c = 0; c < 8; ++c) v[u * 8 + c] = epi_add(v[u * 8 + c], r8[c]);
+                    }
+                } else
                 epi_values<ACT, RES, SCALE, NV>(v, bb, rr, ss, hh);
                 if constexpr (CHK16) {
 #pragma unroll
@@ -636,7 +669,7 @@
                     e.stats_part[(size_t)((n0 + wn * 128) >> 7) * e.ld_part + grow] = make_float2(acc_s, acc_q);
             }
         };
-        auto drain_pass = [&](int p) {
+        auto drain_pass = [&](int p) __attribute__((always_inline)) {
             const bool full = m0 + wm * GEO::WROWS + p * 64 + 64 <= g.M && n0 + wn * 128 + 128 <= g.N;
             if (full) drain(p, std::integral_constant<bool, true>{});
             else drain(p, std::integral_constant<bool, false>{});
@@ -662,7 +695,7 @@
 inline int gemm4d_epi_mode(const GemmArgs<T>& g) {
     const GemmEpilogue<T>& e = g.epi;
     if (e.stats_part && e.residual_lo) {
-        if (sizeof(T) == 2 && e.out_lo && !e.out_f32 && !e.residual && e.act == ACT_NONE && !e.scale && !e.shift && !e.out_f32_b && e.split_col >= g.N &&
+        if (sizeof(T) == 2 && e.out_lo && !e.out_f32 && !e.residual && (e.act == ACT_NONE || e.act == ACT_GELU_TANH) && !e.scale && !e.shift && !e.out_f32_b && e.split_col >= g.N &&
             g.N % 128 == 0 && e.ld_lo % 8 == 0 && e.ld_res_lo % 8 == 0) return G4D_EPI_LN16;
         return -1;
     }
@@ -730,7 +763,9 @@
 template <typename T, bool HALF>
 inline hipError_t launch_gemm4d_mode(const GemmArgs<T>& g, hipStream_t stream, int mode) {
     if (mode == G4D_EPI_F32_LN) return launch_gemm4d_inst<T, ACT_NONE, true, G4D_EPI_F32_LN, HALF>(g, stream);
-    if (mode == G4D_EPI_LN16) return launch_gemm4d_inst<T, ACT_NONE, true, G4D_EPI_LN16, HALF>(g, stream);
+    if (mode == G4D_EPI_LN16)
+        return g.epi.act == ACT_GELU_TANH ? launch_gemm4d_inst<T, ACT_GELU_TANH, true, G4D_EPI_LN16, HALF>(g, stream)
+                                          : launch_gemm4d_inst<T, ACT_NONE, true, G4D_EPI_LN16, HALF>(g, stream);
     if (mode == G4D_EPI_LO_LN) return launch_gemm4d_inst<T, ACT_GELU_TANH, true, G4D_EPI_LO_LN, HALF>(g, stream);
     if (mode == G4D_EPI_F32_SCALE_FOLD) return launch_gemm4d_inst<T, ACT_NONE, false, G4D_EPI_F32_SCALE_FOLD, HALF>(g, stream);
     if (mode == G4D_EPI_F32_SCALE) return launch_gemm4d_inst<T, ACT_NONE, false, G4D_EPI_F32_SCALE, HALF>(g, stream);
diff --git a/zett_amd/csrc/rowops.hip.h b/zett_amd/csrc/rowops.hip.h
--- a/zett_amd/csrc/rowops.hip.h
+++ b/zett_amd/csrc/rowops.hip.h
@@ -776,31 +776,65 @@
     }
 }
 
+__device__ __forceinline__ float2 ln_stats_row(const float2* __restrict__ col, int parts, int ld_part, int H, float eps) {
+    float s = 0.f, q = 0.f;
+    int p = 0;
+    for (; p + 8 <= parts; p += 8) {
+        float2 v[8];
+#pragma unroll
+        for (int j = 0; j < 8; ++j) v[j] = col[(size_t)(p + j) * ld_part];
+#pragma unroll
+        for (int j = 0; j < 8; ++j) { s += v[j].x; q += v[j].y; }
+    }
+    {
+        float2 v[8];
+#pragma unroll
+        for (int j = 0; j < 8; ++j) v[j] = p + j < parts ? col[(size_t)(p + j) * ld_part] : make_float2(0.f, 0.f);
+#pragma unroll
+        for (int j = 0; j < 8; ++j)
+            if (p + j < parts) { s += v[j].x; q += v[j].y; }
+    }
+    const float mean = s / (float)H;
+    const float var = fmaxf(q / (float)H - mean * mean, 0.f);
+    return make_float2(mean, 1.0f / sqrtf(var + eps));
+}
+
 __global__ __launch_bounds__(64) void ln_stats_kernel(const float2* __restrict__ part, int parts, int ld_part, int rows, int H, float eps,
                                                       float* __restrict__ stats) {
     const int r = blockIdx.x * blockDim.x + threadIdx.x;
     if (r >= rows) return;
-    float s = 0.f, q = 0.f;
-    const float2* col = part + r;
-    int p = 0;
-    for (; p + 8 <= parts; p += 8) {
-        float2 v[8];
-#pragma unroll
-        for (int j = 0; j < 8; ++j) v[j] = col[(size_t)(p + j) * ld_part];
-#pragma unroll
-        for (int j = 0; j < 8; ++j) { s += v[j].x; q += v[j].y; }
-    }
-    {
-        float2 v[8];
-#pragma unroll
-        for (int j = 0; j < 8; ++j) v[j] = p + j < parts ? col[(size_t)(p + j) * ld_part] : make_float2(0.f, 0.f);
-#pragma unroll
-        for (int j = 0; j < 8; ++j)
-            if (p + j < parts) { s += v[j].x; q += v[j].y; }
-    }
-    const float mean = s / (float)H;
-    const float var = fmaxf(q / (float)H - mean * mean, 0.f);
-    *(float2*)(stats + 2 * (size_t)r) = make_float2(mean, 1.0f / sqrtf(var + eps));
+    *(float2*)(stats + 2 * (size_t)r) = ln_stats_row(part + r, parts, ld_part, H, eps);
+}
+
+template <typename T, typename BT = void>
+__global__ __launch_bounds__(256) void readout_stats_kernel(const float2* __restrict__ part, int parts, int ld_part, int rows, int H, float eps,
+                                                            float* __restrict__ stats, const T* __restrict__ x, int ld_x,
+                                                            const float* __restrict__ gamma, const float* __restrict__ beta, LnReadout readout) {
+    static_assert(sizeof(T) == 2, "16-bit residual stream");
+    const int r = blockIdx.x * 4 + (int)threadIdx.x / 64;
+    if (r >= rows) return;
+    const int lane = threadIdx.x & 63;
+    const float2 st = ln_stats_row(part + r, parts, ld_part, H, eps);
+    if (lane == 0) {
+        *(float2*)(stats + 2 * (size_t)r) = st;
+        range_report(readout.range_flag, out_of_range(st.x, ZETT_F32_MAX) | out_of_range(st.y, ZETT_F32_MAX), ZETT_RANGE_BIT_ACTIVATION);
+    }
+    if (!readout.out_bias) return;
+    float dot = 0.f;
+    if (readout.bias_w) {
+        for (int c = lane * 8; c < H; c += 512) {
+            float a[8], g[8], b[8], w[8], o[8];
+            load8<T>(x + (size_t)r * ld_x + c, a);
+            load8<float>(gamma + c, g);
+            load8<float>(beta + c, b);
+            load8<float>(readout.bias_w + c, w);
+#pragma unroll
+            for (int k = 0; k < 8; ++k) o[k] = ln_affine(a[k], st.x, st.y, g[k], b[k]);
+            dot += ((o[0] * w[0] + o[1] * w[1]) + (o[2] * w[2] + o[3] * w[3])) + ((o[4] * w[4] + o[5] * w[5]) + (o[6] * w[6] + o[7] * w[7]));
+        }
+    }
+    const float tot = wave_sum(dot);
+    if (lane == 0) ln_readout_store<BT>(readout, r, readout.bias_w ? tot + readout.bias_b[0] : 0.f);
 }
 
 template <typename T>
diff --git a/zett_amd/csrc/zett_hip.hip b/zett_amd/csrc/zett_hip.hip
--- a/zett_amd/csrc/zett_hip.hip
+++ b/zett_amd/csrc/zett_hip.hip
@@ -47,6 +47,7 @@
     struct Folded { void* w = nullptr; float* c = nullptr; float* b = nullptr; };
     std::vector<Folded> fold_qkv, fold_up;
     Folded fold_head_in, fold_head_out;
+    Folded fold_head1_in, fold_head1_out;
     float* head_one = nullptr;
     float* head_zero = nullptr;
     int ln_fold = 1;
@@ -66,6 +67,8 @@
     int gemm_tail_split = 1;
     int gemm_tile_order = 0;
     int ln_rows8 = 1;
+    int readout_fold = 1;
+    int projector_res_lo = 0;
     int table_lo = 1;
     int gemm_group = 0;
     int gemm4d_min_k = 512;
@@ -455,15 +458,16 @@
     }
     if (h->precision != ZETT_PREC_F32 && c.hidden % 128 == 0) {
         auto fold = [&](const float* w32, size_t N, size_t K, const float* gamma, const float* beta, const float* bias,
-                        zett_hypernet::Folded& f) -> int {
+                        zett_hypernet::Folded& f, int32_t* range_flag = nullptr) -> int {
+            if (!range_flag) range_flag = h->range_word;
             HIP_TRY(hipMalloc(&f.w, N * K * es));
             HIP_TRY(hipMalloc((void**)&f.c, N * 4));
             HIP_TRY(hipMalloc((void**)&f.b, N * 4));
             h->owned.push_back(f.w); h->owned.push_back(f.c); h->owned.push_back(f.b);
             if (h->precision == ZETT_PREC_F16)
-                hipLaunchKernelGGL(fold_weight_kernel<f16_t>, dim3((unsigned)N), dim3(256), 0, 0, w32, (int)K, gamma, beta, bias, (f16_t*)f.w, f.c, f.b, h->range_word);
+                hipLaunchKernelGGL(fold_weight_kernel<f16_t>, dim3((unsigned)N), dim3(256), 0, 0, w32, (int)K, gamma, beta, bias, (f16_t*)f.w, f.c, f.b, range_flag);
             else
-                hipLaunchKernelGGL(fold_weight_kernel<bf16_t>, dim3((unsigned)N), dim3(256), 0, 0, w32, (int)K, gamma, beta, bias, (bf16_t*)f.w, f.c, f.b, h->range_word);
+                hipLaunchKernelGGL(fold_weight_kernel<bf16_t>, dim3((unsigned)N), dim3(256), 0, 0, w32, (int)K, gamma, beta, bias, (bf16_t*)f.w, f.c, f.b, range_flag);
             return 0;
         };
         h->fold_qkv.resize(c.layers); h->fold_up.resize(c.layers);
@@ -489,6 +493,14 @@
             if (c.separate_out && !c.single_head)
                 if (int rc = fold(h->w["output_projection_out.1.weight"].f32, c.n_embd, H, h->w["output_projection_out.0.ln.weight"].f32,
                                   h->w["output_projection_out.0.ln.bias"].f32, h->w["output_projection_out.1.bias"].f32, h->fold_head_out)) return rc;
+            if (c.layers >= 1) {
+                const std::string pl = "model.encoder.layer." + std::to_string(c.layers - 1) + ".output.LayerNorm.";
+                if (int rc = fold(h->w["output_projection.0.dense1.weight"].f32, c.intermediate, H, h->w[pl + "weight"].f32, h->w[pl + "bias"].f32,
+                                  h->w["output_projection.0.dense1.bias"].f32, h->fold_head1_in, h->range_word + 1)) return rc;
+                if (c.separate_out && !c.single_head)
+                    if (int rc = fold(h->w["output_projection_out.0.dense1.weight"].f32, c.intermediate, H, h->w[pl + "weight"].f32, h->w[pl + "bias"].f32,
+                                      h->w["output_projection_out.0.dense1.bias"].f32, h->fold_head1_out, h->range_word + 1)) return rc;
+            }
             std::vector<float> ones(w0, 1.0f), zeros(w0, 0.0f);
             HIP_TRY(hipMalloc((void**)&h->head_one, w0 * 4));
             HIP_TRY(hipMalloc((void**)&h->head_zero, w0 * 4));
@@ -499,7 +511,12 @@
         HIP_TRY(hipDeviceSynchronize());
         (void)hipFree(tmp);
     }
-    HIP_TRY(hipMemcpy(h->range_host, h->range_word, 4, hipMemcpyDeviceToHost));
+    HIP_TRY(hipMemcpy(h->range_host, h->range_word, 8, hipMemcpyDeviceToHost));
+    if (h->range_host[1]) {
+        h->fold_head1_in = zett_hypernet::Folded{};
+        h->fold_head1_out = zett_hypernet::Folded{};
+        HIP_TRY(hipMemset(h->range_word + 1, 0, 4));
+    }
     if (h->range_host[0] & ZETT_RANGE_WEIGHT)
         return fail(ZETT_E_RANGE, "a GEMM weight (or a LayerNorm-folded weight W*gamma) exceeds the half range (|w| > 65504 or not finite): "
                                   "this checkpoint needs ZETT_PREC_BF16 or ZETT_PREC_F32");
@@ -557,6 +574,10 @@
         h->ln_rows8 = value != 0;
     } else if (k == "table_lo") {
         h->table_lo = value != 0;
+    } else if (k == "readout_fold") {
+        h->readout_fold = value != 0;
+    } else if (k == "projector_res_lo") {
+        h->projector_res_lo = value != 0;
     } else if (k == "gemm_group") {
         if (value < 0 || value > 64) return fail(ZETT_E_INVALID, "gemm_group must be 0 (default: 4) .. 64");
         h->gemm_group = (int)value;
@@ -1063,14 +1084,43 @@
         check("ln_stats");
     }
 
+    void readout_stats(const float2* parts, int ld_part, int rows, float eps, float* stats, const T* x_lo, const float* gamma, const float* beta,
+                       const LnReadout& readout, int bias_dtype) {
+        if (rc || rows <= 0) return;
+        if constexpr (sizeof(T) == 2) {
+            const int H = h->cfg.hidden;
+            const dim3 grid((rows + 3) / 4);
+#define ZETT_READOUT_STATS(BT) hipLaunchKernelGGL((readout_stats_kernel<T, BT>), grid, dim3(256), 0, st, parts, H / 128, ld_part, rows, H, eps, stats, x_lo, H, gamma, beta, readout)
+            if (bias_dtype < 0) ZETT_READOUT_STATS(void);
+            else if (bias_dtype == ZETT_F16) ZETT_READOUT_STATS(f16_t);
+            else if (bias_dtype == ZETT_BF16) ZETT_READOUT_STATS(bf16_t);
+            else ZETT_READOUT_STATS(float);
+#undef ZETT_READOUT_STATS
+            check("readout_stats");
+        } else {
+            rc = fail(ZETT_E_STATE, "readout_stats needs the 16-bit residual stream");
+        }
+    }
+
+    struct ProjLo { const zett_hypernet::Folded* w1; const float* stats; const float* gamma; const float* beta; };
+
     void projector(const std::string& p, const T* x_lo, const float* x_f32, int rows, T* big, float* pre, float* of, T* ol,
-                   float2* fold_parts = nullptr, int ld_part = 0, float* fold_stats = nullptr) {
+                   float2* fold_parts = nullptr, int ld_part = 0, float* fold_stats = nullptr, const ProjLo* lo = nullptr) {
         const zett_config& c = h->cfg;
+        if (lo && !fold_parts && !rc) { rc = fail(ZETT_E_STATE, "the 16-bit-residual ProjectorBlock is a LayerNorm-fold producer"); return; }
         GemmEpilogue<T> e1 = epi();
         e1.bias = Wf(p + "dense1.bias"); e1.act = ACT_GELU_TANH; e1.out_lo = big; e1.ld_lo = c.intermediate;
-        gemm(x_lo, c.hidden, Wlo(p + "dense1.weight"), c.hidden, rows, c.intermediate, c.hidden, e1);
+        const T* w1 = Wlo(p + "dense1.weight");
+        if (lo && lo->w1) { w1 = (const T*)lo->w1->w; e1.bias = lo->w1->b; e1.fold_stats = lo->stats; e1.fold_c = lo->w1->c; }
+        gemm(x_lo, c.hidden, w1, c.hidden, rows, c.intermediate, c.hidden, e1);
         GemmEpilogue<T> e2 = epi();
-        e2.bias = Wf(p + "dense2.bias"); e2.act = ACT_GELU_TANH; e2.residual = x_f32; e2.ld_res = c.hidden;
+        e2.bias = Wf(p + "dense2.bias"); e2.act = ACT_GELU_TANH;
+        if (lo) {
+            e2.residual_lo = x_lo; e2.ld_res_lo = c.hidden;
+            e2.res_stats = lo->stats; e2.res_gamma = lo->gamma; e2.res_beta = lo->beta;
+        } else {
+            e2.residual = x_f32; e2.ld_res = c.hidden;
+        }
         e2.ld_f32 = c.hidden;
         if (fold_parts) { e2.out_lo = ol; e2.ld_lo = c.hidden; e2.stats_part = fold_parts; e2.ld_part = ld_part; }
         else e2.out_f32 = pre;
@@ -1104,9 +1154,12 @@
         else launch_gather<T, 2>(st, id_list, s0, m, src, c, fb, in_w, in_b, X0, h->range_word);
         R.check("gather_src");
         GemmEpilogue<T> e0 = R.epi();
-        e0.bias = R.Wf("input_projection.0.bias"); e0.out_f32 = Zf; e0.ld_f32 = H; e0.out_lo = Zt; e0.ld_lo = H;
+        const bool res_lo = table_lo && h->projector_res_lo != 0;
+        const typename Runner<T>::ProjLo plo{nullptr, nullptr, nullptr, nullptr};
+        e0.bias = R.Wf("input_projection.0.bias"); e0.out_f32 = res_lo ? nullptr : Zf; e0.ld_f32 = H; e0.out_lo = Zt; e0.ld_lo = H;
         R.gemm(X0, EIN, R.Wlo("input_projection.0.weight"), EIN, m, H, EIN, e0);
-        if (table_lo) R.projector("input_projection.1.", Zt, Zf, m, BIG, PRE, nullptr, tbl16 + (size_t)s0 * H, PARTS, (int)MCS, tblst + 2 * (size_t)s0);
+        if (res_lo) R.projector("input_projection.1.", Zt, nullptr, m, BIG, PRE, nullptr, tbl16 + (size_t)s0 * H, PARTS, (int)MCS, tblst + 2 * (size_t)s0, &plo);
+        else if (table_lo) R.projector("input_projection.1.", Zt, Zf, m, BIG, PRE, nullptr, tbl16 + (size_t)s0 * H, PARTS, (int)MCS, tblst + 2 * (size_t)s0);
         else R.projector("input_projection.1.", Zt, Zf, m, BIG, PRE, tbl32 + (size_t)s0 * H, nullptr);
     }
 }
@@ -1442,6 +1495,14 @@
                      c.predict_bias ? R.Wf("bias_projection.bias") : (const float*)nullptr, bias_out};
         ro.bias_rows = bias_rows;
         ro.range_flag = h->range_word;
+        const bool fold_heads = fold && h->ln_fold == 1 && h->fold_head_in.w != nullptr;
+        const bool two_heads = c.separate_out && !c.single_head;
+        const bool readout_fold = fold_heads && lo_stream && h->readout_fold != 0 && h->fold_head1_in.w != nullptr &&
+                                  (!two_heads || h->fold_head1_out.w != nullptr);
+        float* const head_stats = readout_fold ? other_stats(hs_stats) : STa;
+        if (readout_fold)
+            R.readout_stats(PARTS, (int)ld_parts, rows, c.ln_eps_encoder, hs_stats, Zt, hs_gamma, hs_beta, ro, bias_dtype);
+        else
         R.layernorm(hs_sum, rows, hs_gamma, hs_beta, c.ln_eps_encoder, Cf, Ct, nullptr, ro,
                     lo_stream ? (const T*)Zt : (const T*)nullptr, bias_dtype);
         R.check("readout");
@@ -1451,15 +1512,16 @@
             if (ev_mode == 1 || ev_mode == 3) HIP_TRY(hipEventRecord(h->out_ready[ZETT_OUT_BIAS], st));
         }
 
-        const bool fold_heads = fold && h->ln_fold == 1 && h->fold_head_in.w != nullptr;
+        const typename Runner<T>::ProjLo plo_in{&h->fold_head1_in, hs_stats, hs_gamma, hs_beta}, plo_out{&h->fold_head1_out, hs_stats, hs_gamma, hs_beta};
         {
-            if (fold_heads) R.projector("output_projection.0.", Ct, Cf, rows, BIG, PRE, nullptr, CTX, PARTS, (int)ld_parts, STa);
+            if (readout_fold) R.projector("output_projection.0.", Zt, nullptr, rows, BIG, PRE, nullptr, CTX, PARTS, (int)ld_parts, head_stats, &plo_in);
+            else if (fold_heads) R.projector("output_projection.0.", Ct, Cf, rows, BIG, PRE, nullptr, CTX, PARTS, (int)ld_parts, STa);
             else R.projector("output_projection.0.", Ct, Cf, rows, BIG, PRE, nullptr, CTX);
             GemmEpilogue<T> e = R.epi();
             e.bias = fold_heads ? h->fold_head_in.b : R.Wf("output_projection.1.bias");
             e.scale = c.rescale ? h->head_scale : (fold_heads ? h->head_one : nullptr);
             e.shift = c.rescale ? h->head_shift : (fold_heads ? h->head_zero : nullptr);
-            if (fold_heads) { e.fold_stats = STa; e.fold_c = h->fold_head_in.c; }
+            if (fold_heads) { e.fold_stats = head_stats; e.fold_c = h->fold_head_in.c; }
             e.ld_f32 = E; e.range_final = 1;
             const int width = c.single_head ? EIN : E;
             const bool split = c.single_head && c.separate_out;
@@ -1483,13 +1545,14 @@
             }
         }
         if (c.separate_out && !c.single_head) {
-            if (fold_heads) R.projector("output_projection_out.0.", Ct, Cf, rows, BIG, PRE, nullptr, CTX, PARTS, (int)ld_parts, STa);
+            if (readout_fold) R.projector("output_projection_out.0.", Zt, nullptr, rows, BIG, PRE, nullptr, CTX, PARTS, (int)ld_parts, head_stats, &plo_out);
+            else if (fold_heads) R.projector("output_projection_out.0.", Ct, Cf, rows, BIG, PRE, nullptr, CTX, PARTS, (int)ld_parts, STa);
             else R.projector("output_projection_out.0.", Ct, Cf, rows, BIG, PRE, nullptr, CTX);
             GemmEpilogue<T> e = R.epi();
             e.bias = fold_heads ? h->fold_head_out.b : R.Wf("output_projection_out.1.bias");
             e.scale = c.rescale ? R.Wf("out_scaler.w") : (fold_heads ? h->head_one : nullptr);
             e.shift = c.rescale ? R.Wf("out_scaler.b") : (fold_heads ? h->head_zero : nullptr);
-            if (fold_heads) { e.fold_stats = STa; e.fold_c = h->fold_head_out.c; }
+            if (fold_heads) { e.fold_stats = head_stats; e.fold_c = h->fold_head_out.c; }
             e.ld_f32 = E; e.range_final = 1;
             const T* w2 = fold_heads ? (const T*)h->fold_head_out.w : R.Wlo("output_projection_out.1.weight");
             if (dest) {
```

Measured after the change: 620,800, median of 2. About the same (+0.3%).
